# Moon0shang/HandPoseEstimation-with-3D-CNNs

Hardware: AMD Instinct MI355X
Metric: depth frames/sec to 32^3 TSDF (higher is better)
Workload: dtype f64

## Files before the change

handposeestimation-with-3d-cnns_amd/__init__.py:

```python
from . import _lib
from ._lib import TsdfCam, TsdfError, default_cam
from .voxelize import (AabbBatch, AugmentedStep, CloudGridBatch, MapGridBatch, ObbBatch, PointCloudBatch, PoseError, ProcessAugBatch, ProcessBatch, TsdfBatch,
                       aabb,
                       aug_state, aug_xforms, aug_xforms_at, cloud_grids, denormalize_joints, empty_batch,
                       frames_within, joints_within, normalize_joints, point_clouds, pose_error, process_batch, process_batch_aug,
                       project_joints, release_stream, transform_joints, voxel_pixels, voxelize_aug_grid,
                       voxelize, voxelize_aug, voxelize_grid, voxelize_indexed, voxelize_labels, widen_depth16,
                       invert_xforms, obb_xforms, voxelize_obb, narrow_volumes, voxelize_grid_lowp, voxelize_lowp,
                       map_grids, voxelize_aug_lowp, voxelize_map_grid_lowp, MapStepBatch, compose_xforms, map_step_head,
                       HandCrops, locate_hands, voxelize_frames)
from .pca import JointPCA, fit_joint_pca
from . import augment, dataset, export, packing, pca, shard, synth
from .dataset import MSRA_Dataset, MSRADepthDataset, ResidentLoader, VoxelBatch, VoxelLoader
from .tsdf_numba import cal_tsdf_cuda
from .tsdf_for import tsdf_cal, tsdf_f
from .process import DataProcess

__all__ = ["voxelize", "voxelize_labels", "voxelize_indexed", "ResidentLoader", "voxel_pixels", "release_stream", "voxelize_grid", "voxelize_aug", "augment", "aabb", "TsdfBatch", "AabbBatch", "TsdfCam", "TsdfError",
           "default_cam", "cal_tsdf_cuda", "tsdf_f", "tsdf_cal", "DataProcess", "packing", "shard",
           "synth", "dataset", "MSRADepthDataset", "MSRA_Dataset", "VoxelLoader", "VoxelBatch", "normalize_joints", "denormalize_joints",
           "pca", "JointPCA", "fit_joint_pca", "project_joints", "pose_error", "PoseError", "joints_within", "frames_within",
           "point_clouds", "PointCloudBatch", "cloud_grids", "CloudGridBatch", "process_batch", "ProcessBatch", "aug_xforms",
           "aug_xforms_at", "aug_state", "AugmentedStep", "voxelize_aug_grid", "transform_joints", "process_batch_aug",
           "ProcessAugBatch", "widen_depth16", "obb_xforms", "voxelize_obb", "invert_xforms", "ObbBatch",
           "voxelize_grid_lowp", "voxelize_lowp", "narrow_volumes", "map_grids", "MapGridBatch", "voxelize_map_grid_lowp",
           "voxelize_aug_lowp", "compose_xforms", "map_step_head", "MapStepBatch", "locate_hands", "voxelize_frames",
           "HandCrops"]
```

handposeestimation-with-3d-cnns_amd/_lib.py:

```python
from __future__ import annotations

import contextlib
import ctypes
import os
from typing import NamedTuple

_HERE = os.path.dirname(os.path.abspath(__file__))
_DEFAULT_LIB = os.path.join(_HERE, "libtsdf_hip.so")


def _lib_path() -> str:
    over = os.environ.get("TSDF_HIP_LIB")
    if not over or os.path.abspath(over) == _DEFAULT_LIB:
        return _DEFAULT_LIB
    if os.environ.get("TSDF_ALLOW_LIB_OVERRIDE") != "1":
        raise ImportError(f"TSDF_HIP_LIB={over} asks for a library other than {_DEFAULT_LIB}; set "
                          "TSDF_ALLOW_LIB_OVERRIDE=1 as well if that is intended (experiments only)")
    return over


LIB_PATH = _lib_path()

TSDF_LAYOUT_CZYX = 0
TSDF_LAYOUT_CXYZ = 1
LAYOUTS = {"czyx": TSDF_LAYOUT_CZYX, "cxyz": TSDF_LAYOUT_CXYZ}

TSDF_OK = 0
TSDF_FRAME_OK = 0
TSDF_FRAME_DEGENERATE = 1
TSDF_FRAME_BAD_HEADER = 2


class TsdfError(RuntimeError):
    """A tsdf_* entry point returned a negative status."""


class TsdfCam(ctypes.Structure):

    _fields_ = [
        ("focal", ctypes.c_double),
        ("cx", ctypes.c_double),
        ("cy", ctypes.c_double),
        ("invalid_eps", ctypes.c_float),
        ("trunc_voxels", ctypes.c_float),
    ]


class TsdfLabels(ctypes.Structure):

    _fields_ = [
        ("d_gt", ctypes.c_void_p),
        ("n_joints", ctypes.c_int),
        ("clamp", ctypes.c_int),
        ("d_out_gt_nor", ctypes.c_void_p),
        ("d_out_gt_aug", ctypes.c_void_p),
    ]


class TsdfPca(ctypes.Structure):

    _fields_ = [
        ("d_mean", ctypes.c_void_p),
        ("d_coeff", ctypes.c_void_p),
        ("n_components", ctypes.c_int),
        ("d_out_gt_pca", ctypes.c_void_p),
    ]


ABI_VERSION = 7
INLINE_INDEX_MAX = 32

DEBUG_LIB_PATH = os.path.join(os.path.dirname(_HERE), "build", "libtsdf_hip_debug.so")

AUGMENT_LIB_PATH = os.path.join(_HERE, "libtsdf_augment.so")
AUGMENT_VERSION = 1

AUGSTEP_LIB_PATH = os.path.join(_HERE, "libtsdf_augstep.so")
AUGSTEP_VERSION = 1

AUGGRID_LIB_PATH = os.path.join(_HERE, "libtsdf_auggrid.so")
AUGGRID_VERSION = 1

DEPTH16_LIB_PATH = os.path.join(_HERE, "libtsdf_depth16.so")
DEPTH16_VERSION = 1
DEPTH16_MAX_SHIFT = 7

OBB_LIB_PATH = os.path.join(_HERE, "libtsdf_obb.so")
OBB_VERSION = 1

LOWP_LIB_PATH = os.path.join(_HERE, "libtsdf_lowp.so")
LOWP_VERSION = 1
TSDF_LOWP_F16 = 1
TSDF_LOWP_BF16 = 2

MAPLOWP_LIB_PATH = os.path.join(_HERE, "libtsdf_maplowp.so")
MAPLOWP_VERSION = 1

MAPSTEP_LIB_PATH = os.path.join(_HERE, "libtsdf_mapstep.so")
MAPSTEP_VERSION = 1

LOCATE_LIB_PATH = os.path.join(_HERE, "libtsdf_locate.so")
LOCATE_VERSION = 1
TSDF_LOCATE_F32 = 0
TSDF_LOCATE_U16 = 1


class _Ext(NamedTuple):
    path: str
    version_symbol: str
    version: int
    entries: dict


_vp, _i, _i64, _u64 = ctypes.c_void_p, ctypes.c_int, ctypes.c_int64, ctypes.c_uint64

_EXTS = {
    "augment": _Ext(AUGMENT_LIB_PATH, "tsdf_augment_version", AUGMENT_VERSION, {
        "tsdf_aug_draw_hip": [_vp, _i64, _vp, _i, _u64, _u64, _vp, _vp, _vp, _vp],
    }),
    "augstep": _Ext(AUGSTEP_LIB_PATH, "tsdf_augstep_version", AUGSTEP_VERSION, {
        "tsdf_aug_draw_at_hip": [_vp, _i64, _vp, _i, _vp, _vp, _vp, _vp, _vp, _vp],
    }),
    "auggrid": _Ext(AUGGRID_LIB_PATH, "tsdf_auggrid_version", AUGGRID_VERSION, {
        "tsdf_voxelize_aug_grid_hip": [_vp, _i64, _vp, _vp, _i, _i, ctypes.POINTER(TsdfCam), _i, _vp, _vp, _vp, _vp, _vp],
        "tsdf_transform_joints_hip": [_vp, _vp, _i, _i, _vp, _vp],
    }),
    "depth16": _Ext(DEPTH16_LIB_PATH, "tsdf_depth16_version", DEPTH16_VERSION, {
        "tsdf_depth16_widen_hip": [_vp, _i64, _i, _vp, _vp],
        "tsdf_depth16_host_gather": [_vp, _i64, _vp, _i64, _vp, _i64, _vp, _i64, _vp, _i],
    }),
    "obb": _Ext(OBB_LIB_PATH, "tsdf_obb_version", OBB_VERSION, {
        "tsdf_obb_xforms_hip": [_vp, _i64, _vp, _vp, _i, ctypes.POINTER(TsdfCam), _vp, _vp, _vp, _vp],
    }),
    "lowp": _Ext(LOWP_LIB_PATH, "tsdf_lowp_version", LOWP_VERSION, {
        "tsdf_voxelize_grid_lowp_hip": [_vp, _i64, _vp, _vp, _i64, _vp, _i, _i, ctypes.POINTER(TsdfCam), _i, _i, _vp, _vp,
                                        _vp, _vp],
        "tsdf_lowp_narrow_hip": [_vp, _i64, _i, _vp, _vp],
    }),
    "maplowp": _Ext(MAPLOWP_LIB_PATH, "tsdf_maplowp_version", MAPLOWP_VERSION, {
        "tsdf_map_place_hip": [_vp, _i64, _vp, _vp, _i64, _vp, _i, _i, ctypes.POINTER(TsdfCam), _vp, _vp, _vp, _vp, _vp, _vp],
        "tsdf_voxelize_map_grid_lowp_hip": [_vp, _i64, _vp, _vp, _i64, _vp, _i, _i, ctypes.POINTER(TsdfCam), _i, _i, _vp, _vp,
                                            _vp, _vp, _vp],
    }),
    "mapstep": _Ext(MAPSTEP_LIB_PATH, "tsdf_mapstep_version", MAPSTEP_VERSION, {
        "tsdf_compose_xforms_hip": [_vp, _vp, _i64, _vp, _i, _vp, _vp],
        "tsdf_map_step_head_hip": [_vp, _i64, _vp, _vp, _i64, _vp, _i, _i, ctypes.c_double, ctypes.c_double, ctypes.c_double,
                                   ctypes.c_float, ctypes.c_float, _vp, _vp, _vp, _vp, _vp, _i, _i, _vp, _vp, _vp, _vp, _vp,
                                   _vp, _vp, _vp, _vp, _vp],
    }),
    "locate": _Ext(LOCATE_LIB_PATH, "tsdf_locate_version", LOCATE_VERSION, {
        "tsdf_locate_capacity": [_i, _i, ctypes.c_float, ctypes.c_float, ctypes.c_double, ctypes.POINTER(_i64)],
        "tsdf_locate_hip": [_vp, _i, _i, _i64, _i, _i, _vp, _i, ctypes.c_float, ctypes.c_float, ctypes.c_float,
                            ctypes.c_float, _i, _i, ctypes.c_double, ctypes.c_double, ctypes.c_double, ctypes.c_float,
                            ctypes.c_float, _i64, _vp, _vp, _vp, _vp, _vp, _vp, _vp, _vp, _vp, _vp],
    }),
}

_lib = None
_debug_lib = None
_ext_libs = {}


def _declare(L, entries: dict) -> None:
    for name, argtypes in entries.items():
        fn = getattr(L, name)
        fn.restype = ctypes.c_int
        fn.argtypes = argtypes


def _bind(L, path: str, debug: bool = False):
    vp = ctypes.c_void_p
    cam_p = ctypes.POINTER(TsdfCam)
    L.tsdf_version.restype = ctypes.c_int
    L.tsdf_version.argtypes = []
    if L.tsdf_version() != ABI_VERSION:
        raise ImportError(f"{path} has ABI version {L.tsdf_version()}, this package needs {ABI_VERSION}: rebuild it")
    L.tsdf_strerror.restype = ctypes.c_char_p
    L.tsdf_strerror.argtypes = [ctypes.c_int]
    L.tsdf_resolution_supported.restype = ctypes.c_int
    L.tsdf_resolution_supported.argtypes = [ctypes.c_int]
    L.tsdf_default_cam.restype = None
    L.tsdf_default_cam.argtypes = [cam_p]
    lab_p, pca_p = ctypes.POINTER(TsdfLabels), ctypes.POINTER(TsdfPca)
    i, i64 = ctypes.c_int, ctypes.c_int64
    pack = [vp, i64, vp, vp, i, i, cam_p, i, vp]
    indexed = [vp, i64, vp, vp, i64, vp, i, i, cam_p, i, vp]
    outs = [vp, vp, vp, vp]
    entries = {
            "tsdf_voxelize_hip": pack + outs,
            "tsdf_voxelize_labels_hip": pack + outs + [lab_p],
            "tsdf_voxelize_grid_hip": pack + [vp, vp, vp],
            "tsdf_voxelize_aug_hip": pack + [vp] + outs,
            "tsdf_voxelize_aug_labels_hip": pack + [vp] + outs + [lab_p],
            "tsdf_voxelize_labels_pca_hip": pack + [vp] + outs + [lab_p, pca_p],
            "tsdf_aabb_hip": pack[:7] + [vp] + [vp, vp, vp, vp],
            "tsdf_voxelize_indexed_hip": indexed + outs + [lab_p],
            "tsdf_voxelize_indexed_host_hip": indexed + outs + [lab_p],
            "tsdf_voxelize_indexed_aug_hip": indexed + [vp] + outs + [lab_p],
            "tsdf_voxelize_indexed_pca_hip": indexed + [vp] + outs + [lab_p, pca_p],
            "tsdf_voxelize_indexed_host_pca_hip": indexed + outs + [lab_p, pca_p],
            "tsdf_host_gather_frames": [vp, vp, i64, vp, i64, vp, i64, vp, i],
            "tsdf_host_gather_frames_n": [vp, i64, vp, i64, vp, i64, vp, i64, vp, i],
            "tsdf_normalize_joints_hip": [vp, vp, vp, i, i, i, vp, vp],
            "tsdf_denormalize_joints_hip": [vp, vp, vp, i, i, vp, vp],
            "tsdf_stream_release": [vp],
            "tsdf_project_joints_hip": [vp, vp, vp, i, i, pca_p, vp],
            "tsdf_pose_error_hip": [vp, pca_p, vp, vp, vp, i, i, vp, vp, vp, vp, vp],
            "tsdf_point_clouds_hip": pack[:4] + [i, i, cam_p, ctypes.c_uint64, i64, vp, vp, vp, vp, vp],
            "tsdf_cloud_grid_hip": [vp, i, i, i, cam_p, vp, vp, vp, vp, vp, vp],
            "tsdf_describe_launch": [i, i, i, i, ctypes.c_char_p, i],
            "tsdf_debug_pixmap_hip": pack + [vp, vp, vp, vp],
            "tsdf_debug_set_queue_word": [vp, ctypes.c_uint64],
    }
    _declare(L, {k: v for k, v in entries.items() if debug or not k.startswith("tsdf_debug_")})
    return L


def load():
    global _lib
    if _lib is not None:
        return _lib
    if not os.path.exists(LIB_PATH):
        raise ImportError(
            f"{LIB_PATH} not found: build it with `python -c 'import __graft_entry__ as g; g.build()'` "
            "or `make -C handposeestimation-with-3d-cnns_amd/csrc`. There is no CPU fallback."
        )
    _lib = _bind(ctypes.CDLL(LIB_PATH), LIB_PATH)
    return _lib


def load_debug():
    global _debug_lib
    if _debug_lib is not None:
        return _debug_lib
    if not os.path.exists(DEBUG_LIB_PATH):
        raise ImportError(f"{DEBUG_LIB_PATH} not found: build it with `make -C handposeestimation-with-3d-cnns_amd/csrc debug` "
                          "(__graft_entry__.build() does)")
    L = _bind(ctypes.CDLL(DEBUG_LIB_PATH), DEBUG_LIB_PATH, debug=True)
    _debug_lib = L
    return L


def _load_ext(name: str):
    L = _ext_libs.get(name)
    if L is not None:
        return L
    ext = _EXTS[name]
    if not os.path.exists(ext.path):
        raise ImportError(f"{ext.path} not found: build it with `make -C handposeestimation-with-3d-cnns_amd/csrc "
                          f"{name}` (__graft_entry__.build() does). There is no CPU fallback.")
    L = ctypes.CDLL(ext.path)
    _declare(L, {ext.version_symbol: [], **ext.entries})
    have = getattr(L, ext.version_symbol)()
    if have != ext.version:
        raise ImportError(f"{ext.path} has version {have}, this package needs {ext.version}: rebuild it")
    _ext_libs[name] = L
    return L


def load_augment():
    return _load_ext("augment")


def load_augstep():
    return _load_ext("augstep")


def load_auggrid():
    return _load_ext("auggrid")


def load_depth16():
    return _load_ext("depth16")


def load_obb():
    return _load_ext("obb")


def load_lowp():
    return _load_ext("lowp")


def load_maplowp():
    return _load_ext("maplowp")


def load_mapstep():
    return _load_ext("mapstep")


def load_locate():
    return _load_ext("locate")


@contextlib.contextmanager
def using_debug_library():
    global _lib
    prev = _lib
    _lib = load_debug()
    try:
        yield _lib
    finally:
        _lib = prev


def check(status: int, what: str):
    if status != TSDF_OK:
        msg = load().tsdf_strerror(status).decode()
        raise TsdfError(f"{what}: {msg} (status {status})")


def default_cam() -> TsdfCam:
    c = TsdfCam()
    load().tsdf_default_cam(ctypes.byref(c))
    return c
```

handposeestimation-with-3d-cnns_amd/dataset.py:

```python
from __future__ import annotations

import ctypes
import os
import sys
import queue
import threading
import warnings
from typing import Iterator, List, NamedTuple, Optional, Sequence, Tuple, Union

import numpy as np
import torch
import torch.utils.data as data

from . import _lib, augment, packing, shard
from .pca import JointPCA, fit_joint_pca
from .voxelize import (AugmentedStep, TsdfBatch, _get_raw_stream, aabb, aug_state, aug_xforms, aug_xforms_at,
                       denormalize_joints, empty_batch, normalize_joints, obb_xforms, project_joints, voxelize,
                       voxelize_aug, voxelize_grid_lowp, voxelize_indexed, voxelize_labels, widen_depth16, _lowp_dtype)


def _common_depth_shift(packs: Sequence[packing.PackedFrames]) -> Optional[int]:
    forms = sorted({-1 if pk.depth_shift is None else int(pk.depth_shift) for pk in packs})
    if len(forms) > 1:
        names = ", ".join("float32" if f < 0 else f"16-bit with shift {f}" for f in forms)
        raise ValueError(f"the packs of one dataset must share one depth form, these are {names}: repack them "
                         "(packing.pack_tree(..., depth16=None) or one forced shift, overwrite=True)")
    return None if not forms or forms[0] < 0 else forms[0]


def _subset(size: str) -> Tuple[int, int]:
    if size == "full":
        return 9, 17
    if size == "small":
        return 4, 5
    raise ValueError("size must be 'full' or 'small'")


class MSRADepthDataset(data.Dataset):

    def __init__(self, root_path: str, train: bool = True, test_idx: int = 2, size: str = "full",
                 subjects: Optional[Sequence[str]] = None, packed_dir: Optional[str] = None,
                 build_packs: bool = True):
        n_sub, n_ges = _subset(size)
        self.root_path = root_path
        self.train = train
        self.test_idx = test_idx
        if subjects is not None:
            all_sub = list(subjects)
        elif root_path is not None and os.path.isdir(root_path):
            skip = os.path.abspath(packed_dir) if packed_dir is not None else None
            all_sub = sorted(d for d in os.listdir(root_path) if os.path.isdir(os.path.join(root_path, d))
                             and os.path.abspath(os.path.join(root_path, d)) != skip)[:n_sub]
        elif packed_dir is not None:
            all_sub = sorted(f[:-7] for f in os.listdir(packed_dir) if f.endswith(".tsdfpk"))[:n_sub]
        else:
            raise ValueError("root_path is not a directory and no packed_dir was given")
        if not 0 <= test_idx < len(all_sub):
            raise ValueError("test_idx out of range")
        chosen = [s for i, s in enumerate(all_sub) if (i != test_idx) == train]
        self.subjects = chosen
        self.paths: List[str] = []
        self.packs: List[packing.PackedFrames] = []
        self._pack_of = np.zeros(0, np.int32)
        self._local = np.zeros(0, np.int64)
        gts: List[np.ndarray] = []
        if packed_dir is not None:
            pk_of, loc = [], []
            for sub in chosen:
                path = os.path.join(packed_dir, sub + ".tsdfpk")
                if not os.path.exists(path):
                    if not build_packs:
                        raise FileNotFoundError(path)
                    packing.pack_tree(root_path, packed_dir, subjects=[sub])
                pk = packing.PackedFrames.load(path, mmap=True)
                gs = pk.group_start if pk.group_start is not None else np.array([0, len(pk)])
                end = int(gs[min(n_ges, len(gs) - 1)])
                self.packs.append(pk)
                pk_of.append(np.full(end, len(self.packs) - 1, np.int32))
                loc.append(np.arange(end, dtype=np.int64))
                gts.append(np.asarray(pk.gt[:end]) if pk.gt is not None else np.zeros((end, 63), np.float32))
            if pk_of:
                self._pack_of, self._local = np.concatenate(pk_of), np.concatenate(loc)
        else:
            for sub in chosen:
                sub_dir = os.path.join(root_path, sub)
                gestures = sorted(g for g in os.listdir(sub_dir) if os.path.isdir(os.path.join(sub_dir, g)))
                for ges in gestures[:n_ges]:
                    g_dir = os.path.join(sub_dir, ges)
                    bin_num, gt = packing.read_joint(g_dir)
                    self.paths += packing.gesture_bin_paths(g_dir, bin_num)
                    gts.append(gt)
        self.depth_shift = _common_depth_shift(self.packs)
        self.ground_truth = np.concatenate(gts) if gts else np.zeros((0, 63), np.float32)

    @classmethod
    def from_packs(cls, packs: Sequence[packing.PackedFrames]) -> "MSRADepthDataset":
        self = cls.__new__(cls)
        self.root_path, self.train, self.test_idx, self.subjects, self.paths = None, True, -1, [], []
        self.packs = list(packs)
        self.depth_shift = _common_depth_shift(self.packs)
        self._pack_of = np.concatenate([np.full(len(pk), k, np.int32) for k, pk in enumerate(self.packs)])
        self._local = np.concatenate([np.arange(len(pk), dtype=np.int64) for pk in self.packs])
        self.ground_truth = np.concatenate([np.asarray(pk.gt) if pk.gt is not None else np.zeros((len(pk), 63), np.float32)
                                            for pk in self.packs])
        return self

    @property
    def packed(self) -> bool:
        return bool(self.packs)

    def __len__(self) -> int:
        return len(self._local) if self.packed else len(self.paths)

    def pixels(self) -> Optional[np.ndarray]:
        if not self.packed:
            return None
        out = np.empty(len(self), np.int64)
        for k, pk in enumerate(self.packs):
            m = self._pack_of == k
            out[m] = pk.pixels[self._local[m]]
        return out

    def __getitem__(self, index: int):
        if self.packed:
            pk = self.packs[int(self._pack_of[index])]
            h, d = pk.frame(int(self._local[index]))
            return np.asarray(h), np.asarray(d), self.ground_truth[index]
        header, depth = packing.read_bin(self.paths[index])
        return header, depth, self.ground_truth[index]

    def pin_packs(self, limit_bytes: int = 32 << 30) -> bool:
        if not self.packed or sum(int(pk.depth.nbytes) for pk in self.packs) > limit_bytes:
            return False
        for pk in self.packs:
            pk.pin()
        return True

    def contiguous_source(self, idx: np.ndarray):
        idx = np.asarray(idx, np.int64)
        if not self.packed or idx.size == 0 or not (np.diff(idx) == 1).all():
            return None
        ks = self._pack_of[idx]
        pk = self.packs[int(ks[0])]
        if ks[0] != ks[-1] or getattr(pk, "_pinned", None) is None:
            return None
        a, b = int(self._local[idx[0]]), int(self._local[idx[-1]]) + 1
        view = pk.slice(a, b)
        view.gt = self.ground_truth[idx]
        return pk._pinned[int(pk.offsets[a]):int(pk.offsets[b])], view

    def take(self, idx: np.ndarray, depth_out: Optional[np.ndarray] = None) -> packing.PackedFrames:
        idx = np.asarray(idx, np.int64)
        if self.packed and idx.size:
            ks = self._pack_of[idx]
            if (ks == ks[0]).all():
                out = self.packs[int(ks[0])].take(self._local[idx], depth_out)
                out.gt = self.ground_truth[idx]
                return out
            if self.depth_shift is not None:
                raw = [self.packs[int(k)].raw_frame(int(l)) for k, l in zip(ks, self._local[idx])]
                off = np.zeros(idx.size + 1, np.int64)
                np.cumsum([d.size for _, d in raw], out=off[1:])
                if depth_out is not None and depth_out.dtype != np.uint16:
                    raise TypeError(f"depth_out is {depth_out.dtype}, the dataset's packs hold uint16 depth")
                depth = depth_out[: off[-1]] if depth_out is not None else np.empty(int(off[-1]), np.uint16)
                for k, (_, d) in enumerate(raw):
                    depth[off[k]:off[k + 1]] = d
                return packing.PackedFrames(depth, off, np.stack([np.asarray(h) for h, _ in raw]), self.ground_truth[idx],
                                            depth_shift=self.depth_shift)
            pk = packing.pack_frames(self.packs[int(k)].frame(int(l)) for k, l in zip(ks, self._local[idx]))
            if depth_out is not None:
                depth_out[: pk.depth.size] = pk.depth
                pk.depth = depth_out[: pk.depth.size]
            pk.gt = self.ground_truth[idx]
            return pk
        pk = packing.pack_frames(self[int(i)][:2] for i in idx)
        if depth_out is not None:
            depth_out[: pk.depth.size] = pk.depth
            pk.depth = depth_out[: pk.depth.size]
        pk.gt = self.ground_truth[idx] if idx.size else np.zeros((0, 63), np.float32)
        return pk


def collate_frames(batch) -> Tuple[packing.PackedFrames, np.ndarray]:
    pk = packing.pack_frames((h, d) for h, d, _ in batch)
    gt = np.stack([g for _, _, g in batch]).astype(np.float32) if batch else np.zeros((0, 63), np.float32)
    return pk, gt


def voxelize_batch(pk: packing.PackedFrames, gt: np.ndarray, device, res: int = 32, pin: bool = True):
    depth, offsets, headers = pk.to_torch(device, pin=pin, non_blocking=True)
    tgt = torch.from_numpy(np.ascontiguousarray(gt))
    if pin:
        tgt = tgt.pin_memory()
    tgt = tgt.to(device, non_blocking=True)
    out: TsdfBatch = voxelize(depth, offsets, headers, res=res)
    return out.tsdf, tgt, out.max_l, out.mid_p, out.status


class VoxelBatch(NamedTuple):

    tsdf: torch.Tensor
    gt: torch.Tensor
    max_l: torch.Tensor
    mid_p: torch.Tensor
    status: torch.Tensor
    gt_nor: Optional[torch.Tensor]


def plan_batches(n: int, batch_size: int, rank: int = 0, world: int = 1, shuffle: bool = False, seed: int = 0,
                 epoch: int = 0, drop_last: bool = False, weights: Optional[np.ndarray] = None,
                 balance: Optional[str] = None) -> List[np.ndarray]:
    if balance is None:
        balance = "pixels" if weights is not None else "frames"
    if balance not in ("frames", "pixels"):
        raise ValueError("balance must be 'frames' or 'pixels'")
    if balance == "pixels" and weights is None:
        raise ValueError("balance='pixels' needs the per-frame weights")
    bounds = shard.shard_bounds(n, world, weights if balance == "pixels" else None)
    if not 0 <= rank < world:
        raise ValueError("rank out of range")
    a, b = bounds[rank]
    idx = np.arange(a, b, dtype=np.int64)
    if shuffle:
        np.random.default_rng((seed, epoch, rank)).shuffle(idx)
    if balance == "frames":
        if n < world:
            raise ValueError(f"balance='frames' needs at least one frame per rank (n={n}, world={world})")
        lens = [e - s for s, e in bounds]
        if not drop_last and idx.size < max(lens):
            idx = np.concatenate([idx, idx[:1]])
    batches = [idx[i:i + batch_size] for i in range(0, idx.size, batch_size)]
    if balance == "frames":
        if drop_last:
            batches = batches[: min(lens) // batch_size]
    elif drop_last and batches and batches[-1].size < batch_size:
        batches.pop()
    return batches


class _Staging:

    def __init__(self, max_px: int, bs: int, device, with_gt: bool, depth16: bool = False):
        self.h_depth = torch.empty(max_px, dtype=torch.uint16 if depth16 else torch.float32).pin_memory()
        self.d_depth16 = torch.empty(max_px, dtype=torch.uint16, device=device) if depth16 else None
        self.h_off = torch.empty(bs + 1, dtype=torch.int64).pin_memory()
        self.h_hdr = torch.empty((bs, 6), dtype=torch.int32).pin_memory()
        self.h_gt = torch.empty((bs, 63), dtype=torch.float32).pin_memory() if with_gt else None
        self.d_depth = torch.empty(max_px, dtype=torch.float32, device=device)
        self.copied = torch.cuda.Event()
        self.consumed = torch.cuda.Event()
        self.filled = threading.Event()
        self.free = threading.Event()
        self.free.set()
        self.used = False
        self.n = 0
        self.npx = 0
        self.src = None


class _BatchLoader:

    def __init__(self, dataset: MSRADepthDataset, batch_size: int, device, res, shuffle, seed, drop_last, rank, world,
                 labels, clamp, layout, balance):
        self.balance = balance
        self.ds, self.bs, self.device, self.res = dataset, int(batch_size), torch.device(device), res
        self.shuffle, self.seed, self.drop_last = shuffle, seed, drop_last
        self.rank, self.world = rank, world
        self.labels, self.clamp, self.layout = labels, clamp, layout
        self.epoch = 0

    def _batches(self) -> List[np.ndarray]:
        return plan_batches(len(self.ds), self.bs, self.rank, self.world, self.shuffle, self.seed, self.epoch,
                            self.drop_last, self.ds.pixels() if self.balance == "pixels" else None, self.balance)

    def __len__(self) -> int:
        return len(self._batches())


class VoxelLoader(_BatchLoader):

    def __init__(self, dataset: MSRADepthDataset, batch_size: int, device, res: int = 32,
                 shuffle: bool = False, seed: int = 0, drop_last: bool = False,
                 rank: int = 0, world: int = 1, labels: bool = True, clamp: bool = True,
                 max_pixels: Optional[int] = None, layout: str = "czyx", pin_packs: bool = True,
                 balance: str = "frames"):
        super().__init__(dataset, batch_size, device, res, shuffle, seed, drop_last, rank, world, labels, clamp, layout,
                         balance)
        self.max_px = int(max_pixels) if max_pixels else self.bs * 320 * 240
        self.pin_packs = pin_packs
        self._sets: Optional[List[_Staging]] = None
        self._copy_stream = None

    def __iter__(self) -> Iterator[VoxelBatch]:
        batches = self._batches()
        self.epoch += 1
        if self._sets is None:
            self._sets = [_Staging(self.max_px, self.bs, self.device, True, getattr(self.ds, "depth_shift", None) is not None)
                          for _ in range(2)]
            if self.pin_packs:
                self.ds.pin_packs()
        sets = self._sets
        shift = getattr(self.ds, "depth_shift", None)
        for s in sets:
            if s.used:
                s.consumed.synchronize()
            s.free.set()
            s.filled.clear()
            s.used = False
        err: "queue.Queue" = queue.Queue()
        stop = threading.Event()

        def work():
            try:
                for k, b in enumerate(batches):
                    s = sets[k & 1]
                    while not s.free.wait(0.05):
                        if stop.is_set():
                            return
                    s.free.clear()
                    if s.used:
                        s.consumed.synchronize()
                    direct = self.ds.contiguous_source(b)
                    if direct is not None:
                        s.src, pk = direct
                    else:
                        pk = self.ds.take(b, s.h_depth.numpy())
                        s.src = s.h_depth[: pk.depth.size]
                    if pk.depth.size > self.max_px:
                        raise ValueError(f"batch of {pk.depth.size} pixels exceeds max_pixels={self.max_px}")
                    s.n, s.npx = len(pk), int(pk.depth.size)
                    s.h_off.numpy()[: s.n + 1] = pk.offsets
                    s.h_hdr.numpy()[: s.n] = pk.headers
                    s.h_gt.numpy()[: s.n] = pk.gt
                    s.filled.set()
            except BaseException as e:
                err.put(e)
                for s in sets:
                    s.filled.set()

        t = threading.Thread(target=work, daemon=True)
        t.start()
        if self._copy_stream is None:
            self._copy_stream = torch.cuda.Stream(device=self.device)
        copy_stream = self._copy_stream
        try:
            for k in range(len(batches)):
                cur = torch.cuda.current_stream(self.device)
                s = sets[k & 1]
                s.filled.wait()
                if not err.empty():
                    raise err.get()
                s.filled.clear()
                n, npx = s.n, s.npx
                with torch.cuda.stream(copy_stream):
                    if k >= 2:
                        copy_stream.wait_event(s.consumed)
                    if shift is None:
                        s.d_depth[:npx].copy_(s.src, non_blocking=True)
                    else:
                        s.d_depth16[:npx].copy_(s.src, non_blocking=True)
                        widen_depth16(s.d_depth16[:npx], shift, out=s.d_depth[:npx])
                    s.copied.record(copy_stream)
                cur.wait_event(s.copied)
                out, gt_nor, gt = voxelize_labels(s.d_depth[:npx], s.h_off[: n + 1], s.h_hdr[:n], s.h_gt[:n], res=self.res,
                                                  layout=self.layout, clamp=self.clamp, gt_copy=True)
                if not self.labels:
                    gt_nor = None
                s.consumed.record(cur)
                s.used = True
                s.free.set()
                yield VoxelBatch(out.tsdf, gt, out.max_l, out.mid_p, out.status, gt_nor)
        finally:
            stop.set()
            t.join()


class ResidentPacks:

    def __init__(self, dataset: MSRADepthDataset, device):
        if not dataset.packed:
            raise ValueError("a resident dataset needs packs (packing.pack_tree + packed_dir=, or from_packs)")
        packs = dataset.packs
        px = np.array([int(pk.depth.size) for pk in packs], np.int64)
        nf = np.array([len(pk) for pk in packs], np.int64)
        pbase = np.concatenate([[0], np.cumsum(px)])
        fbase = np.concatenate([[0], np.cumsum(nf)])
        self.depth = torch.empty(int(pbase[-1]), dtype=torch.float32, device=device)
        with warnings.catch_warnings():
            warnings.simplefilter("ignore", UserWarning)
            for k, pk in enumerate(packs):
                dst = self.depth[int(pbase[k]):int(pbase[k + 1])]
                if pk.depth_shift is None:
                    dst.copy_(torch.from_numpy(np.ascontiguousarray(pk.depth)))
                else:
                    tmp = torch.from_numpy(np.ascontiguousarray(pk.depth)).to(self.depth.device)
                    widen_depth16(tmp, pk.depth_shift, out=dst)
                    del tmp
        off = np.concatenate([np.asarray(pk.offsets[:-1], np.int64) + pbase[k] for k, pk in enumerate(packs)]
                             + [pbase[-1:]])
        hdr = np.concatenate([np.asarray(pk.headers, np.int32).reshape(-1, 6) for pk in packs])
        gt = np.concatenate([np.asarray(pk.gt, np.float32).reshape(len(pk), -1) if pk.gt is not None
                             else np.zeros((len(pk), 63), np.float32) for pk in packs])
        self.offsets = torch.from_numpy(off).to(device)
        self.headers = torch.from_numpy(np.ascontiguousarray(hdr)).to(device)
        self.gt = torch.from_numpy(np.ascontiguousarray(gt)).to(device)
        self.frame = fbase[dataset._pack_of] + dataset._local

    def nbytes(self) -> int:
        return 4 * self.depth.numel()


class ResidentLoader(_BatchLoader):

    def __init__(self, dataset: MSRADepthDataset, batch_size: int, device, res: int = 32, shuffle: bool = False,
                 seed: int = 0, drop_last: bool = False, rank: int = 0, world: int = 1, labels: bool = True,
                 clamp: bool = True, layout: str = "czyx", augment: Union[bool, str] = False, balance: str = "frames",
                 prefetch: int = 1, ring: int = 2, graph: bool = False, frame: str = "camera",
                 volume_dtype: Optional[torch.dtype] = None):
        if frame not in ("camera", "obb"):
            raise ValueError(f"frame must be 'camera' or 'obb', got {frame!r}")
        if frame == "obb" and (augment or graph):
            raise ValueError("frame='obb' does not combine with augment or graph=True (the two maps are not composed)")
        if volume_dtype is not None:
            _lowp_dtype(volume_dtype)
            if augment or graph or frame == "obb":
                raise ValueError("volume_dtype does not combine with augment, frame='obb' or graph=True (the low-precision "
                                 "voxel pass is the plain one)")
        if not dataset.packed:
            raise ValueError("ResidentLoader needs a pack-backed dataset (packing.pack_tree + packed_dir=, or from_packs)")
        if prefetch < 1 or ring < 2:
            raise ValueError("prefetch must be >= 1 and ring >= 2")
        if isinstance(augment, str) and augment != "device":
            raise ValueError(f"augment must be False, True or 'device', got {augment!r}")
        if graph is not False and graph is not True:
            raise ValueError(f"graph must be False or True, got {graph!r}")
        if graph and (augment != "device" or prefetch != 1):
            raise ValueError("graph=True replays the augmented step: it needs augment='device' and prefetch=1")
        self.augment = bool(augment)
        self.device_draws = augment == "device"
        self.graph = graph
        self.frame = frame
        self.obb = None
        self.obb_status = None
        self._step = None
        self.volume_dtype = volume_dtype
        self._lowp = None
        self._lowp_ring = None
        self._mapped = self.augment or frame == "obb"
        self.prefetch, self.ring = int(prefetch), int(ring)
        super().__init__(dataset, batch_size, device, res, shuffle, seed, drop_last, rank, world, labels, clamp, layout,
                         balance)
        self._dev = None
        self._g = None
        self._idx = None
        self._blocks = None

    def resident_bytes(self) -> int:
        return sum(4 * int(pk.depth.size) for pk in self.ds.packs)

    def _upload(self):
        rp = ResidentPacks(self.ds, self.device)
        self._dev = (rp.depth, rp.offsets, rp.headers, rp.gt)
        self._g = rp.frame
        pin = self.bs > _lib.INLINE_INDEX_MAX or self._mapped
        self._idx = [(torch.empty(self.bs, dtype=torch.int64).pin_memory() if pin else torch.empty(self.bs, dtype=torch.int64),
                      torch.cuda.Event()) for _ in range(2)]
        self._used = [False, False]
        self._mid = None
        if self.frame == "obb":
            ob = obb_xforms(rp.depth, rp.offsets, rp.headers)
            self.obb, self.obb_status = ob.xforms, ob.status
        if self.volume_dtype is not None:
            ab = aabb(rp.depth, rp.offsets, rp.headers, res=self.res)
            rows = torch.cat([ab.ori, ab.grid[:, 4:6], torch.zeros_like(ab.ori)], dim=1)
            self._lowp = (rows, ab.grid[:, 3].contiguous(), ab.grid[:, :3].contiguous(), ab.status)
        if self.augment:
            mid = aabb(rp.depth, rp.offsets, rp.headers, res=self.res).grid[:, :3]
            if self.device_draws:
                self._mid = mid.contiguous()
                self._xf = torch.empty((self.ring if self.prefetch > 1 else 2, self.bs * self.prefetch, 24),
                                       dtype=torch.float64, device=self.device)
            else:
                self._mid = mid.cpu().numpy().astype(np.float64)
                self._xf = [torch.empty((self.bs, 24), dtype=torch.float64).pin_memory() for _ in range(2)]

    def __iter__(self) -> Iterator[VoxelBatch]:
        batches = self._batches()
        self.epoch += 1
        if self._dev is None:
            self._upload()
        if self.volume_dtype is not None:
            return self._iter_lowp(batches)
        if self.prefetch > 1:
            return self._iter_blocks(batches, self.epoch)
        return self._iter_single(batches, self.epoch)

    def _iter_lowp(self, batches) -> Iterator[VoxelBatch]:
        depth, off, hdr, gt = self._dev
        rows, max_l, mid_p, status = self._lowp
        if not batches:
            return
        bs, P, R = self.bs, self.prefetch, self.res
        if P > 1 and self._lowp_ring is None:
            self._lowp_ring = [torch.empty((bs * P, 3, R, R, R), dtype=self.volume_dtype, device=self.device)
                               for _ in range(self.ring)]
        d_idx = torch.from_numpy(np.ascontiguousarray(self._g[np.concatenate(batches)])).to(self.device)
        pos = 0
        for blk, k0 in enumerate(range(0, len(batches), P)):
            mine = batches[k0:k0 + P]
            nfr = int(sum(b.size for b in mine))
            idx = d_idx[pos:pos + nfr]
            pos += nfr
            out = self._lowp_ring[blk % self.ring][:nfr] if P > 1 else None
            tsdf, _ = voxelize_grid_lowp(depth, off, hdr, rows, res=R, layout=self.layout, dtype=self.volume_dtype,
                                         index=idx, out=out)
            ml, mp, st = max_l.index_select(0, idx), mid_p.index_select(0, idx), status.index_select(0, idx)
            g = gt.index_select(0, idx)
            gt_nor = None
            if self.labels:
                gt_nor = normalize_joints(g, ml, mp, clamp=self.clamp)
                bad = (st != _lib.TSDF_FRAME_OK).reshape((-1,) + (1,) * (g.dim() - 1))
                gt_nor = torch.where(bad, torch.full_like(gt_nor, 0.5), gt_nor)
            a = 0
            for b in mine:
                e = a + int(b.size)
                yield VoxelBatch(tsdf[a:e], g[a:e], ml[a:e], mp[a:e], st[a:e], gt_nor[a:e] if self.labels else None)
                a = e

    def _epoch_key(self, epoch: int) -> int:
        return augment.device_key(self.seed, epoch, self.rank) if self.device_draws else 0

    def _host_draw(self, gidx: np.ndarray, batches, epoch: int, k0: int = 0) -> np.ndarray:
        xf = np.empty((gidx.size, 24), np.float64)
        pos = 0
        for k, b in enumerate(batches, k0):
            xf[pos:pos + b.size] = augment.random_affines(self._mid[gidx[pos:pos + b.size]],
                                                          rng=(self.seed, epoch, self.rank, k))[0]
            pos += b.size
        return xf

    def _maps(self, index: torch.Tensor, slot: int, key: int, pos: int, drawn: Optional[torch.Tensor]):
        if self.frame == "obb":
            return self.obb.index_select(0, index)
        if self.device_draws:
            return aug_xforms(self._mid, index=index, key=key, counter0=pos, out=self._xf[slot, :index.numel()])
        return drawn

    def _iter_single(self, batches, epoch) -> Iterator[VoxelBatch]:
        depth, off, hdr, gt = self._dev
        key, pos = self._epoch_key(epoch), 0
        for k, b in enumerate(batches):
            cur = torch.cuda.current_stream(self.device)
            h_idx, done = self._idx[k & 1]
            if self._used[k & 1]:
                done.synchronize()
            n = int(b.size)
            gidx = self._g[b]
            if self.graph and n == self.bs:
                if self._step is None:
                    self._step = AugmentedStep(depth, off, hdr, n, gt=gt, centres=self._mid, res=self.res,
                                               layout=self.layout, clamp=self.clamp)
                out, gt_nor, g = self._step.step(gidx, key, pos)
            else:
                h_idx.numpy()[:n] = gidx
                xf, idx = None, h_idx[:n]
                if self._mapped:
                    drawn = None
                    if self.frame == "obb":
                        idx = idx.to(self.device, non_blocking=True)
                    elif not self.device_draws:
                        h_xf = self._xf[k & 1]
                        h_xf.numpy()[:n] = self._host_draw(gidx, (b,), epoch, k)
                        drawn = h_xf[:n].to(self.device, non_blocking=True)
                    xf = self._maps(idx, k & 1, key, pos, drawn)
                out, gt_nor, g = voxelize_indexed(depth, off, hdr, idx, gt, res=self.res, layout=self.layout,
                                                  clamp=self.clamp, gt_copy=True, xforms=xf)
                done.record(cur)
                self._used[k & 1] = True
            pos += n
            yield VoxelBatch(out.tsdf, g, out.max_l, out.mid_p, out.status, gt_nor if self.labels else None)

    def _make_blocks(self):
        depth, off, hdr, gt = self._dev
        cap, R = self.bs * self.prefetch, self.res
        lab_shape = (cap,) + tuple(gt.shape[1:])
        blocks = []
        for _ in range(self.ring):
            out = empty_batch(cap, R, self.device)
            gt_nor = torch.empty(lab_shape, dtype=torch.float32, device=self.device)
            g = torch.empty(lab_shape, dtype=torch.float32, device=self.device)
            views = [self._view(out, gt_nor, g, j * self.bs, (j + 1) * self.bs) for j in range(self.prefetch)]
            blocks.append((out, gt_nor, g, views))
        return blocks

    def _view(self, out, gt_nor, g, a, b) -> VoxelBatch:
        return VoxelBatch(out.tsdf[a:b], g[a:b], out.max_l[a:b], out.mid_p[a:b], out.status[a:b],
                          gt_nor[a:b] if self.labels else None)

    def _iter_blocks(self, batches, epoch) -> Iterator[VoxelBatch]:
        depth, off, hdr, gt = self._dev
        if self._blocks is None:
            self._blocks = self._make_blocks()
        if not batches:
            return
        bs, P = self.bs, self.prefetch
        flat = np.concatenate(batches)
        gidx = self._g[flat]
        d_idx = torch.from_numpy(np.ascontiguousarray(gidx)).to(self.device)
        key = self._epoch_key(epoch)
        d_xf = None
        if self.augment and not self.device_draws:
            d_xf = torch.from_numpy(self._host_draw(gidx, batches, epoch)).to(self.device)
        pos = 0
        for blk, k0 in enumerate(range(0, len(batches), P)):
            mine = batches[k0:k0 + P]
            nfr = int(sum(b.size for b in mine))
            out, gt_nor, g, views = self._blocks[blk % self.ring]
            full = nfr == bs * P
            if full:
                o, gn, gg = out, gt_nor, g
            else:
                o = TsdfBatch(out.tsdf[:nfr], out.max_l[:nfr], out.mid_p[:nfr], out.status[:nfr])
                gn, gg = gt_nor[:nfr], g[:nfr]
            idx, xf = d_idx[pos:pos + nfr], None
            if self._mapped:
                xf = self._maps(idx, blk % self.ring, key, pos, None if d_xf is None else d_xf[pos:pos + nfr])
            voxelize_indexed(depth, off, hdr, idx, gt, res=self.res, layout=self.layout, clamp=self.clamp,
                             out=o, out_gt_nor=gn, out_gt=gg, xforms=xf)
            pos += nfr
            if full:
                yield from views
            else:
                a = 0
                for b in mine:
                    yield self._view(out, gt_nor, g, a, a + int(b.size))
                    a += int(b.size)


class PreBatched:

    __slots__ = ("batch",)

    def __init__(self, batch):
        self.batch = batch


def _collate_prebatched(batch, *, collate_fn_map=None):
    return batch[0].batch


try:
    from torch.utils.data._utils.collate import default_collate_fn_map as _collate_map
    _collate_map[PreBatched] = _collate_prebatched
except ImportError:
    _collate_map = None


class _SlotGuard:

    __slots__ = ("batch", "_stor", "_cdata", "_base")

    def __init__(self, batch):
        self.batch = batch
        self._stor = tuple(t.untyped_storage() for t in batch)
        self._cdata = tuple(s._cdata for s in self._stor)
        self._base = None

    def counts(self):
        rc, uc, b, c = sys.getrefcount, _storage_use_count, self.batch, self._cdata
        if len(c) == 5:
            return (rc(b), rc(b[0]), rc(b[1]), rc(b[2]), rc(b[3]), rc(b[4]), uc(c[0]), uc(c[1]), uc(c[2]), uc(c[3]),
                    uc(c[4]))
        return (rc(b), rc(b[0]), rc(b[1]), rc(b[2]), rc(b[3]), uc(c[0]), uc(c[1]), uc(c[2]), uc(c[3]))

    def arm(self):
        self._base = self.counts()

    def held(self) -> bool:
        return self.counts() != self._base


_storage_use_count = getattr(torch._C, "_storage_Use_Count", None)
_guard_ok: Optional[bool] = None


def _slot_guard_works() -> bool:
    global _guard_ok
    if _guard_ok is None:
        ok = _storage_use_count is not None
        if ok:
            try:
                holder = [PreBatched(tuple(torch.zeros(2, 3) for _ in range(4)))]
                g = _SlotGuard(holder[0].batch)
                g.arm()
                ok = not g.held()
                for make in (lambda b: b, lambda b: b[1], lambda b: b[0][:, 1], lambda b: b[2].detach(), lambda b: b[3].data,
                             lambda b: b[0].numpy()):
                    ref = make(holder[0].batch)
                    ok = ok and g.held()
                    del ref
                    ok = ok and not g.held()
            except Exception:
                ok = False
        _guard_ok = bool(ok)
    return _guard_ok


class MSRA_Dataset(data.Dataset):

    def __init__(self, root_path, opt=None, train=True, aug=False, device="cuda", block: int = 1024,
                 packed_dir: Optional[str] = None, resident: Optional[bool] = None, prebatched: Optional[bool] = None,
                 ring: Optional[int] = None, aug_seed: int = 0, _raw: Optional[MSRADepthDataset] = None, pca=None):
        if isinstance(aug, str) and aug != "device":
            raise ValueError(f"aug must be False, True or 'device', got {aug!r}")
        self.AUG = bool(aug)
        self.aug_device = aug == "device"
        self.aug_seed = aug_seed
        self.size = getattr(opt, "size", "small")
        self.test_idx = int(getattr(opt, "test_index", 2))
        self.PCA_SZ = int(getattr(opt, "PCA_SZ", 63))
        self.train = train
        self.raw = _raw if _raw is not None else MSRADepthDataset(root_path, train=train, test_idx=self.test_idx,
                                                                  size=self.size, packed_dir=packed_dir)
        self.device = torch.device(device)
        self.block = int(block)
        self._cache_block = -1
        self._cache: Optional[TsdfBatch] = None
        self._cache_gt: Optional[torch.Tensor] = None
        self._last = -1
        self.resident = self.raw.packed if resident is None else bool(resident)
        self.prebatched = (self.resident and _collate_map is not None) if prebatched is None else bool(prebatched)
        if self.prebatched and not self.resident:
            raise ValueError("prebatched=True needs a resident (pack-backed) dataset")
        self._ring_req = ring
        self._rp: Optional[ResidentPacks] = None
        self._fast = None
        self._n = len(self.raw)
        self._aug_params = None
        self._xf_table = None
        self._aug_key = 0
        self._aug_state = None
        self._aug_mid = None
        if self.aug_device:
            self._aug_key = augment.device_key(aug_seed, 0, 0)
        elif self.AUG:
            self._aug_params = augment.draw_params(self._n, aug_seed)
        self.pca = None
        self._cache_pca: Optional[torch.Tensor] = None
        if pca is not None and pca is not False:
            if pca is True:
                if not train:
                    raise ValueError("pca=True fits on a TRAINING dataset; pass the training set's basis (its .pca, a "
                                     "JointPCA or a path) to a test dataset")
                basis = fit_joint_pca(self)
            elif isinstance(pca, JointPCA):
                basis = pca
            else:
                basis = JointPCA.load(os.fspath(pca))
            basis.check_k(self.PCA_SZ)
            self.pca = basis.to(self.device)
            self.PCA_mean, self.PCA_coeff = basis.torch_decode_args(self.PCA_SZ, self.device)

    @classmethod
    def from_raw(cls, raw: MSRADepthDataset, device="cuda", **kw) -> "MSRA_Dataset":
        return cls(None, device=device, _raw=raw, **kw)

    def __len__(self):
        return 2 * self._n if self.AUG else self._n

    def _resident_packs(self) -> "ResidentPacks":
        if self._rp is None:
            self._rp = ResidentPacks(self.raw, self.device)
            if self.AUG:
                rp = self._rp
                mid = aabb(rp.depth, rp.offsets, rp.headers).grid[:, :3]
                self._frame2 = np.ascontiguousarray(np.concatenate([rp.frame, rp.frame]))
                if self.aug_device:
                    self._aug_mid = mid.contiguous()
                    self._draw_frame = np.ascontiguousarray(np.concatenate([np.full(self._n, -1, np.int64), rp.frame]))
                    self._draw_counter = np.ascontiguousarray(np.tile(np.arange(self._n, dtype=np.int64), 2))
                else:
                    mid = mid.cpu().numpy().astype(np.float64)[rp.frame]
                    self._xf_table = np.ascontiguousarray(np.concatenate(
                        [augment.identity_affines(self._n), augment.affines_from_params(mid, *self._aug_params)]))
        return self._rp

    def _device_state(self) -> torch.Tensor:
        if self._aug_state is None:
            self._aug_state = aug_state(self._aug_key, 0, self.device)
        return self._aug_state

    def _device_maps(self, idx: np.ndarray) -> torch.Tensor:
        return aug_xforms_at(self._aug_mid, self._device_state(),
                             index=torch.from_numpy(self._draw_frame[idx]).to(self.device),
                             counters=torch.from_numpy(self._draw_counter[idx]).to(self.device))

    def _voxelize_items(self, idx: np.ndarray, clamp: bool = True):
        dev = self.device
        kw = {} if self.pca is None else {"pca": self.pca, "k": self.PCA_SZ}
        if self.resident:
            rp = self._resident_packs()
            xf = None
            if self.aug_device:
                xf = self._device_maps(idx)
            elif self.AUG:
                xf = torch.from_numpy(self._xf_table[idx]).to(dev)
            frame = self._frame2 if self.AUG else rp.frame
            r = voxelize_indexed(rp.depth, rp.offsets, rp.headers, torch.from_numpy(frame[idx]).to(dev), rp.gt,
                                 clamp=clamp, gt_copy=True, xforms=xf, **kw)
            return r[0], r[2], r[1], (r[3] if kw else None)
        src = idx % self._n
        pk = self.raw.take(src)
        depth, offsets, headers = pk.to_torch(dev, pin=False, non_blocking=False)
        gt = torch.from_numpy(np.ascontiguousarray(pk.gt)).to(dev)
        if not self.AUG:
            if not kw:
                return voxelize(depth, offsets, headers, res=32), gt, None, None
            out, gt_nor, gt_pca = voxelize_labels(depth, offsets, headers, gt, res=32, clamp=clamp, **kw)
            return out, gt, gt_nor, gt_pca
        mid = aabb(depth, offsets, headers).grid[:, :3]
        if self.aug_device:
            pos = np.where(idx < self._n, -1, np.arange(idx.size)).astype(np.int64)
            xf = aug_xforms_at(mid.contiguous(), self._device_state(), index=torch.from_numpy(pos).to(dev),
                               counters=torch.from_numpy(np.ascontiguousarray(src, np.int64)).to(dev))
        else:
            xf = augment.affines_from_params(mid.cpu().numpy().astype(np.float64), *(p[src] for p in self._aug_params))
            plain = idx < self._n
            xf[plain] = augment.identity_affines(int(plain.sum()))
            xf = torch.from_numpy(xf).to(dev)
        out, gt_nor, gt_aug = voxelize_aug(depth, offsets, headers, xf, res=32, gt=gt, clamp=clamp)
        gt_pca = project_joints(gt_aug, out.max_l, out.mid_p, self.pca, self.PCA_SZ) if kw else None
        return out, gt_aug, gt_nor, gt_pca

    def _fit_labels(self) -> np.ndarray:
        n, dev, us = self._n, self.device, []
        if self.resident:
            rp = self._resident_packs()
            ab = aabb(rp.depth, rp.offsets, rp.headers)
            fr = torch.from_numpy(rp.frame).to(dev)
            grid, st, gt = ab.grid[fr], ab.status[fr], rp.gt[fr]
            u = normalize_joints(gt.contiguous(), grid[:, 3].contiguous(), grid[:, :3].contiguous(), clamp=False)
            us.append(u[st == 0].cpu().numpy())
        else:
            for a in range(0, n, self.block):
                pk = self.raw.take(np.arange(a, min(n, a + self.block)))
                depth, offsets, headers = pk.to_torch(dev, pin=False, non_blocking=False)
                ab = aabb(depth, offsets, headers)
                gt = torch.from_numpy(np.ascontiguousarray(pk.gt)).to(dev)
                u = normalize_joints(gt, ab.grid[:, 3].contiguous(), ab.grid[:, :3].contiguous(), clamp=False)
                us.append(u[ab.status == 0].cpu().numpy())
        for a in range(n, len(self), self.block):
            out, _, u, _ = self._voxelize_items(np.arange(a, min(len(self), a + self.block)), clamp=False)
            us.append(u[out.status == 0].cpu().numpy())
        return np.concatenate(us) if us else np.zeros((0, 63), np.float32)

    def _tuples(self, out, gt, gt_pca, m: int):
        if gt_pca is None:
            return [(out.tsdf[k], gt[k], out.max_l[k], out.mid_p[k]) for k in range(m)]
        return [(out.tsdf[k], gt[k], out.max_l[k], out.mid_p[k], gt_pca[k]) for k in range(m)]

    def _load_block(self, blk: int):
        a, b = blk * self.block, min(len(self.raw), (blk + 1) * self.block)
        self._cache, self._cache_gt, _, self._cache_pca = self._voxelize_items(np.arange(a, b))
        self._cache_block = blk

    class _Fast:

        kGroup = 16
        pca, k = None, 0

        def __init__(self, rp: "ResidentPacks", bs: int, ring: int, device, frame=None, xf_table=None, pca=None, k=0,
                     draw=None):
            self._ctypes, self._lib = ctypes, _lib
            self.always_fresh = not _slot_guard_works()
            ring = max(2, int(ring))
            self.iring = -(-max(ring, self.kGroup) // self.kGroup) * self.kGroup
            self.bs, self.ring, self.count, self.replaced = bs, ring, 0, 0
            self.L = _lib.load()
            self.pca, self.k = pca, int(k)
            self.rp_gt = rp.gt
            self.nc = rp.gt.shape[1]
            d = torch.device(device)
            self.device = d if d.index is not None else torch.device("cuda", torch.cuda.current_device())
            self.dev_index = self.device.index
            self.h_idx = torch.empty((self.iring, bs), dtype=torch.int64).pin_memory()
            self.h_idx_np = self.h_idx.numpy()
            self.rows = [self.h_idx_np[k] for k in range(self.iring)]
            self.idx_ptrs = [self.h_idx[k].data_ptr() for k in range(self.iring)]
            self.head = (rp.depth.data_ptr(), rp.depth.numel(), rp.offsets.data_ptr(), rp.headers.data_ptr(),
                         int(rp.headers.shape[0]))
            self.slots = [None] * ring
            self.labels = [None] * ring
            self.args = [None] * ring
            self.pcas = [None] * ring
            self.results = [None] * ring
            self.guard = [None] * ring
            for k in range(ring):
                self._fresh(k)
            self.read = [torch.cuda.Event() for _ in range(self.iring // self.kGroup)]
            self.read_used = [False] * (self.iring // self.kGroup)
            self.raw_stream = _get_raw_stream if _get_raw_stream is not None else \
                (lambda i: torch.cuda.current_stream(i).cuda_stream)
            self.cur_dev = getattr(torch._C, "_cuda_getDevice", torch.cuda.current_device)
            self.fn = self.L.tsdf_voxelize_indexed_hip
            self.plain_xf = ()
            if pca is not None:
                self.fn, self.plain_xf = self.L.tsdf_voxelize_indexed_pca_hip, (None,)
            self.take = (rp.frame if frame is None else frame).take
            self.by_value = xf_table is None and draw is None and bs <= _lib.INLINE_INDEX_MAX
            self.fn_host = self.L.tsdf_voxelize_indexed_host_hip if pca is None else \
                self.L.tsdf_voxelize_indexed_host_pca_hip
            self.fn_aug = self.L.tsdf_voxelize_indexed_aug_hip if pca is None else self.L.tsdf_voxelize_indexed_pca_hip
            self.idx_buf = np.empty(bs, np.int64)
            self.idx_ptr = self.idx_buf.ctypes.data
            self.xf_take = None
            if xf_table is not None:
                self.h_xf = torch.empty((self.iring, bs, 24), dtype=torch.float64).pin_memory()
                self.h_xf_np = self.h_xf.numpy()
                self.xf_rows = [self.h_xf_np[k] for k in range(self.iring)]
                self.xf_ptr = [self.h_xf[k].data_ptr() for k in range(self.iring)]
                self.xf_take = xf_table.take
            self.draw = None
            if draw is not None:
                centres, state, frames, counters = draw
                self.fn_draw = _lib.load_augstep().tsdf_aug_draw_at_hip
                self.draw = (centres, state)
                self.draw_head = (centres.data_ptr(), int(centres.shape[0]))
                self.state_ptr = state.data_ptr()
                self.h_draw = torch.empty((self.iring, 2, bs), dtype=torch.int64).pin_memory()
                self.h_draw_np = self.h_draw.numpy()
                self.draw_rows = [(self.h_draw_np[k, 0], self.h_draw_np[k, 1]) for k in range(self.iring)]
                self.draw_ptrs = [(self.h_draw[k, 0].data_ptr(), self.h_draw[k, 1].data_ptr()) for k in range(self.iring)]
                self.d_xf = torch.empty((self.iring, bs, 24), dtype=torch.float64, device=self.device)
                self.xf_ptr = [self.d_xf[k].data_ptr() for k in range(self.iring)]
                self.frame_take, self.counter_take = frames.take, counters.take

        def _fresh(self, k: int) -> None:
            self._alloc(k)
            self.guard[k].arm()

        def _alloc(self, k: int) -> None:
            R, bs, nc, dev = 32, self.bs, self.nc, self.device
            tsdf = torch.empty((bs, 3, R, R, R), dtype=torch.float32, device=dev)
            gt = torch.empty((bs, nc), dtype=torch.float32, device=dev)
            max_l = torch.empty(bs, dtype=torch.float32, device=dev)
            mid_p = torch.empty((bs, 3), dtype=torch.float32, device=dev)
            status = torch.empty(bs, dtype=torch.int32, device=dev)
            gt_nor = torch.empty((bs, nc), dtype=torch.float32, device=dev)
            self.slots[k] = (tsdf, gt, max_l, mid_p, status, gt_nor)
            self.labels[k] = self._lib.TsdfLabels(self.rp_gt.data_ptr(), nc // 3, 1, gt_nor.data_ptr(), gt.data_ptr())
            self.args[k] = (tsdf.data_ptr(), max_l.data_ptr(), mid_p.data_ptr(), status.data_ptr(),
                            self._ctypes.byref(self.labels[k]))
            batch = (tsdf, gt, max_l, mid_p)
            if self.pca is not None:
                gt_pca = torch.empty((bs, self.k), dtype=torch.float32, device=dev)
                mean, coeff = self.pca.device_tensors(dev)
                self.pcas[k] = self._lib.TsdfPca(mean.data_ptr(), coeff.data_ptr(), self.k, gt_pca.data_ptr())
                self.slots[k] = self.slots[k] + (gt_pca,)
                self.args[k] = self.args[k] + (self._ctypes.byref(self.pcas[k]),)
                batch = batch + (gt_pca,)
            self.results[k] = [PreBatched(batch)]
            self.guard[k] = _SlotGuard(self.results[k][0].batch)

        def held(self, k: int) -> bool:
            return self.always_fresh or self.guard[k].held()

        def next_slot(self) -> int:
            k = self.count % self.ring
            if self.held(k):
                self._fresh(k)
                self.replaced += 1
            return k

        def sync(self) -> None:
            torch.cuda.current_stream(self.device).synchronize()

    def _ring_size(self, n: int) -> int:
        if self._ring_req:
            return max(2, int(self._ring_req))
        vol = n * (3 * 32 ** 3 * 4)
        return max(2, min(256, (2 << 30) // max(vol, 1)))

    def _fast_batch(self, indices):
        f = self._fast
        n = len(indices)
        if f is None or n > f.bs:
            if f is not None:
                f.sync()
            f = self._fast = MSRA_Dataset._Fast(self._rp, n, self._ring_size(n), self.device,
                                                frame=self._frame2 if self.AUG else None, xf_table=self._xf_table,
                                                pca=self.pca, k=self.PCA_SZ,
                                                draw=(self._aug_mid, self._device_state(), self._draw_frame,
                                                      self._draw_counter) if self.aug_device else None)
        k = f.next_slot()
        a = f.args[k]
        if f.by_value:
            fn = f.fn_host
            f.idx_buf[:n] = f.take(indices)
            with torch.cuda.device(f.device):
                rc = fn(*f.head, f.idx_ptr, n, 32, None, 0, f.raw_stream(f.dev_index), *a)
        else:
            ki = f.count % f.iring
            within = ki & (f.kGroup - 1)
            if within == 0 and f.read_used[ki >> 4]:
                f.read[ki >> 4].synchronize()
            if n == f.bs:
                f.take(indices, out=f.rows[ki])
            else:
                f.h_idx_np[ki, :n] = f.take(indices)
            if f.draw is not None:
                fr, cn = f.draw_rows[ki]
                if n == f.bs:
                    f.frame_take(indices, out=fr)
                    f.counter_take(indices, out=cn)
                else:
                    fr[:n] = f.frame_take(indices)
                    cn[:n] = f.counter_take(indices)
                with torch.cuda.device(f.device):
                    stream = f.raw_stream(f.dev_index)
                    fn = f.fn_draw
                    rc = fn(*f.draw_head, f.draw_ptrs[ki][0], n, f.state_ptr, f.draw_ptrs[ki][1], stream, f.xf_ptr[ki],
                            None, None)
                    if rc == 0:
                        fn = f.fn_aug
                        rc = fn(*f.head, f.idx_ptrs[ki], n, 32, None, 0, stream, f.xf_ptr[ki], *a)
            elif f.xf_take is not None:
                fn = f.fn_aug
                if n == f.bs:
                    f.xf_take(indices, axis=0, out=f.xf_rows[ki])
                else:
                    f.h_xf_np[ki, :n] = f.xf_take(indices, axis=0)
                with torch.cuda.device(f.device):
                    rc = fn(*f.head, f.idx_ptrs[ki], n, 32, None, 0, f.raw_stream(f.dev_index), f.xf_ptr[ki], *a)
            else:
                fn = f.fn
                if f.cur_dev() == f.dev_index:
                    rc = fn(*f.head, f.idx_ptrs[ki], n, 32, None, 0, f.raw_stream(f.dev_index), *f.plain_xf, *a)
                else:
                    with torch.cuda.device(f.device):
                        rc = fn(*f.head, f.idx_ptrs[ki], n, 32, None, 0, f.raw_stream(f.dev_index), *f.plain_xf, *a)
            if within == f.kGroup - 1:
                f.read[ki >> 4].record(torch.cuda.current_stream(f.device))
                f.read_used[ki >> 4] = True
        if rc != 0:
            _lib.check(rc, fn.__name__)
        f.count += 1
        if n == f.bs:
            return f.results[k]
        return [PreBatched(tuple(t[:n] for t in f.results[k][0].batch))]

    def __getitems__(self, indices):
        if data.get_worker_info() is not None:
            raise RuntimeError("MSRA_Dataset produces its items on the GPU: use it with num_workers=0 (the reference's "
                               "default, train.py:38), there is nothing for loader processes to do")
        f = self._fast
        if f is not None and f.by_value and len(indices) == f.bs and f.cur_dev() == f.dev_index:
            k = f.next_slot()
            f.take(indices, out=f.idx_buf)
            a = f.args[k]
            rc = f.fn_host(*f.head, f.idx_ptr, f.bs, 32, None, 0, f.raw_stream(f.dev_index), *a)
            if rc != 0:
                _lib.check(rc, "tsdf_voxelize_indexed_host_hip")
            f.count += 1
            self._last = indices[-1]
            return f.results[k]
        if self.prebatched:
            if not indices:
                raise IndexError("empty batch")
            self._resident_packs()
            self._last = indices[-1]
            return self._fast_batch(indices)
        idx = np.asarray([int(i) for i in indices], np.int64)
        if idx.size and (idx.min() < 0 or idx.max() >= len(self)):
            raise IndexError(int(idx.max() if idx.max() >= len(self) else idx.min()))
        self._last = int(idx[-1]) if idx.size else self._last
        out, gt, _, gt_pca = self._voxelize_items(idx)
        return self._tuples(out, gt, gt_pca, idx.size)

    def _items_of(self, indices):
        r = self.__getitems__(indices)
        if r and isinstance(r[0], PreBatched):
            b = r[0].batch
            return [tuple(t[k].clone() for t in b) for k in range(len(indices))]
        return r

    def __getitem__(self, index):
        index = int(index)
        if not 0 <= index < len(self):
            raise IndexError(index)
        if self.AUG:
            self._last = index
            return self._items_of([index])[0]
        blk = index // self.block
        if blk != self._cache_block:
            if index != self._last + 1 and index % self.block:
                return self._items_of([index])[0]
            self._load_block(blk)
        self._last = index
        k = index - blk * self.block
        c = self._cache
        if self._cache_pca is not None:
            return c.tsdf[k], self._cache_gt[k], c.max_l[k], c.mid_p[k], self._cache_pca[k]
        return c.tsdf[k], self._cache_gt[k], c.max_l[k], c.mid_p[k]
```

handposeestimation-with-3d-cnns_amd/voxelize.py:

```python
from __future__ import annotations

import ctypes
from typing import NamedTuple, Optional

import torch

from . import _lib


class TsdfBatch(NamedTuple):
    tsdf: torch.Tensor
    max_l: torch.Tensor
    mid_p: torch.Tensor
    status: torch.Tensor


_get_raw_stream = getattr(torch._C, "_cuda_getCurrentRawStream", None)


def _raw_stream(dev) -> int:
    if _get_raw_stream is not None:
        return _get_raw_stream(dev.index)
    return torch.cuda.current_stream(dev).cuda_stream


class _Current:

    __slots__ = ("guard",)

    def __init__(self, dev):
        self.guard = None if torch.cuda.current_device() == dev.index else torch.cuda.device(dev)

    def __enter__(self):
        if self.guard is not None:
            self.guard.__enter__()

    def __exit__(self, *exc):
        if self.guard is not None:
            self.guard.__exit__(*exc)
        return False


def _dev_check(name, t, dtype, device=None, host_ok=False):
    if t.__class__ is torch.Tensor and t.is_cuda and t.dtype is dtype and t.is_contiguous() and \
            (device is None or t.device == device):
        return
    if not isinstance(t, torch.Tensor):
        raise TypeError(f"{name} must be a torch.Tensor")
    if host_ok and not t.is_cuda and t.is_pinned():
        device = None
    elif not t.is_cuda:
        raise ValueError(f"{name} must live on the GPU" + (" or in page-locked host memory" if host_ok else "") +
                         f" (there is no CPU path); got device {t.device}")
    if t.dtype != dtype:
        raise TypeError(f"{name} must be {dtype}, got {t.dtype}")
    if not t.is_contiguous():
        raise ValueError(f"{name} must be contiguous")
    if device is not None and t.device != device:
        raise ValueError(f"{name} is on {t.device}, expected {device}")


def _pack(L, depth, offsets, headers, res=None, layout="czyx"):
    if layout not in _lib.LAYOUTS:
        raise ValueError("layout must be 'czyx' or 'cxyz'")
    _dev_check("depth", depth, torch.float32)
    dev = depth.device
    _dev_check("offsets", offsets, torch.int64, dev, host_ok=True)
    _dev_check("headers", headers, torch.int32, dev, host_ok=True)
    if headers.dim() != 2 or headers.shape[1] != 6:
        raise ValueError("headers must have shape [n, 6]")
    n = headers.shape[0]
    if offsets.numel() != n + 1:
        raise ValueError("offsets must have n+1 entries")
    if res is None:
        return dev, n, None
    if not L.tsdf_resolution_supported(int(res)):
        raise ValueError(f"unsupported grid resolution {res} (multiple of 4 in 4..128)")
    return dev, n, int(res)


def _coords(name, t, rows) -> int:
    if t.shape[0] != rows:
        raise ValueError(f"{name} must have shape [{rows}, 3*J] or [{rows}, J, 3]")
    nc = t.numel() // rows if rows else 0
    if rows and (nc % 3 or not 1 <= nc // 3 <= 170):
        raise ValueError(f"{name} must hold 1..170 joints of 3 coordinates per frame")
    return nc


def _shaped(name, t, shape, dtype, dev):
    _dev_check(name, t, dtype, dev)
    if tuple(t.shape) != shape and (len(shape) != 1 or t.numel() != shape[0]):
        raise ValueError(f"{name} must have shape {shape}")
    return t


def _out(name, t, shape, dtype, dev):
    return torch.empty(shape, dtype=dtype, device=dev) if t is None else _shaped(name, t, shape, dtype, dev)


def empty_batch(n: int, R: int, dev) -> TsdfBatch:
    return TsdfBatch(_out("tsdf", None, (n, 3, R, R, R), torch.float32, dev), _out("max_l", None, (n,), torch.float32, dev),
                     _out("mid_p", None, (n, 3), torch.float32, dev), _out("status", None, (n,), torch.int32, dev))


def _make_out(out, n, R, dev) -> "TsdfBatch":
    if out is None:
        return empty_batch(n, R, dev)
    _dev_check("out.tsdf", out.tsdf, torch.float32, dev)
    _dev_check("out.max_l", out.max_l, torch.float32, dev)
    _dev_check("out.mid_p", out.mid_p, torch.float32, dev)
    _dev_check("out.status", out.status, torch.int32, dev)
    if tuple(out.tsdf.shape) != (n, 3, R, R, R) or out.max_l.numel() != n or \
            tuple(out.mid_p.shape) != (n, 3) or out.status.numel() != n:
        raise ValueError("out tensors have the wrong shape")
    return out


def _cam(cam):
    return ctypes.byref(cam) if cam is not None else None


def _ptr(t):
    return t.data_ptr() if t is not None else None


def _head(depth, offsets, headers, n, R, cam, layout) -> list:
    return [depth.data_ptr(), depth.numel(), offsets.data_ptr(), headers.data_ptr(), n, R, _cam(cam), _lib.LAYOUTS[layout],
            None]


def _call(dev, fn, args: list, stream_at: int) -> None:
    with _Current(dev):
        args[stream_at] = _raw_stream(dev)
        rc = fn(*args)
    _lib.check(rc, fn.__name__)


def _labels_struct(gt, n_src, n, dev, clamp, out_gt_nor=None, out_gt=None, want_gt=False):
    _dev_check("gt", gt, torch.float32, dev, host_ok=True)
    nc = _coords("gt", gt, n_src) or 63
    shape = (n,) + tuple(gt.shape[1:])
    gt_nor = _out("out_gt_nor", out_gt_nor, shape, torch.float32, dev)
    gt_dev = _out("out_gt", out_gt, shape, torch.float32, dev) if want_gt or out_gt is not None else None
    return _lib.TsdfLabels(gt.data_ptr(), nc // 3, 1 if clamp else 0, gt_nor.data_ptr(), _ptr(gt_dev)), gt_nor, gt_dev


def voxelize(depth: torch.Tensor, offsets: torch.Tensor, headers: torch.Tensor, res: int = 32,
             layout: str = "czyx", cam: Optional[_lib.TsdfCam] = None,
             out: Optional[TsdfBatch] = None) -> TsdfBatch:
    L = _lib.load()
    dev, n, R = _pack(L, depth, offsets, headers, res, layout)
    out = _make_out(out, n, R, dev)
    if n:
        _call(dev, L.tsdf_voxelize_hip, _head(depth, offsets, headers, n, R, cam, layout) +
              [out.tsdf.data_ptr(), out.max_l.data_ptr(), out.mid_p.data_ptr(), out.status.data_ptr()], 8)
    return out


def voxelize_labels(depth: torch.Tensor, offsets: torch.Tensor, headers: torch.Tensor, gt: torch.Tensor,
                    res: int = 32, layout: str = "czyx", cam: Optional[_lib.TsdfCam] = None, clamp: bool = True,
                    out: Optional[TsdfBatch] = None, out_gt_nor: Optional[torch.Tensor] = None,
                    gt_copy: bool = False, pca=None, k: Optional[int] = None):
    L = _lib.load()
    dev, n, R = _pack(L, depth, offsets, headers, res, layout)
    out = _make_out(out, n, R, dev)
    lab, gt_nor, gt_dev = _labels_struct(gt, n, n, dev, clamp, out_gt_nor, want_gt=gt_copy)
    pst = gt_pca = None
    if pca is not None:
        pst, gt_pca = _pca_struct(pca, k, n, lab.n_joints, dev)
    if n:
        head = _head(depth, offsets, headers, n, R, cam, layout)
        tail = [out.tsdf.data_ptr(), out.max_l.data_ptr(), out.mid_p.data_ptr(), out.status.data_ptr(), ctypes.byref(lab)]
        if pst is None:
            _call(dev, L.tsdf_voxelize_labels_hip, head + tail, 8)
        else:
            _call(dev, L.tsdf_voxelize_labels_pca_hip, head + [None] + tail + [ctypes.byref(pst)], 8)
    return ((out, gt_nor, gt_dev) if gt_copy else (out, gt_nor)) + ((gt_pca,) if pca is not None else ())


def voxelize_indexed(depth: torch.Tensor, offsets: torch.Tensor, headers: torch.Tensor, index: torch.Tensor,
                     gt: Optional[torch.Tensor] = None, res: int = 32, layout: str = "czyx",
                     cam: Optional[_lib.TsdfCam] = None, clamp: bool = True, out: Optional[TsdfBatch] = None,
                     gt_copy: bool = False, xforms: Optional[torch.Tensor] = None,
                     out_gt_nor: Optional[torch.Tensor] = None, out_gt: Optional[torch.Tensor] = None,
                     pca=None, k: Optional[int] = None):
    L = _lib.load()
    by_value = isinstance(index, torch.Tensor) and not index.is_cuda and not index.is_pinned() and \
        index.dtype is torch.int64 and index.dim() == 1 and index.is_contiguous() and \
        index.numel() <= _lib.INLINE_INDEX_MAX and xforms is None
    if not by_value:
        _dev_check("index", index, torch.int64, depth.device if isinstance(depth, torch.Tensor) else None, host_ok=True)
    if index.dim() != 1:
        raise ValueError("index must have shape [n]")
    dev, n_pack, R = _pack(L, depth, offsets, headers, res, layout)
    n = index.numel()
    out = _make_out(out, n, R, dev)
    lab = gt_nor = gt_dev = None
    if xforms is not None:
        _dev_check("xforms", xforms, torch.float64, dev, host_ok=True)
        if xforms.numel() != 24 * n:
            raise ValueError("xforms must have shape [n, 24] (forward rows then inverse rows)")
    if gt is not None:
        _dev_check("gt", gt, torch.float32, dev, host_ok=True)
        if gt.dim() < 2:
            raise ValueError("gt must hold the labels of every frame of the pack: [N, 3*J] or [N, J, 3]")
        lab, gt_nor, gt_dev = _labels_struct(gt, n_pack, n, dev, clamp, out_gt_nor, out_gt, want_gt=gt_copy)
        gt_copy = gt_dev is not None
    pst = gt_pca = None
    if pca is not None:
        if gt is None:
            raise ValueError("pca= needs gt (the projection is of the batch's labels)")
        pst, gt_pca = _pca_struct(pca, k, n, lab.n_joints, dev)
    if n:
        head = _head(depth, offsets, headers, n, R, cam, layout)
        head[4:5] = [n_pack, index.data_ptr(), n]
        tail = [out.tsdf.data_ptr(), out.max_l.data_ptr(), out.mid_p.data_ptr(), out.status.data_ptr(),
                ctypes.byref(lab) if lab is not None else None]
        if pst is not None:
            if by_value:
                _call(dev, L.tsdf_voxelize_indexed_host_pca_hip, head + tail + [ctypes.byref(pst)], 10)
            else:
                _call(dev, L.tsdf_voxelize_indexed_pca_hip, head + [_ptr(xforms)] + tail + [ctypes.byref(pst)], 10)
        elif by_value:
            _call(dev, L.tsdf_voxelize_indexed_host_hip, head + tail, 10)
        elif xforms is None:
            _call(dev, L.tsdf_voxelize_indexed_hip, head + tail, 10)
        else:
            _call(dev, L.tsdf_voxelize_indexed_aug_hip, head + [xforms.data_ptr()] + tail, 10)
    if gt is None:
        return out
    return ((out, gt_nor, gt_dev) if gt_copy else (out, gt_nor)) + ((gt_pca,) if pca is not None else ())


def _pca_struct(pca, k, n, n_joints, dev, out=None):
    k = pca.check_k(k)
    if pca.n_coords != 3 * n_joints:
        raise ValueError(f"the PCA basis is for {pca.n_coords} coordinates, the labels have {3 * n_joints}")
    mean, coeff = pca.device_tensors(dev)
    out = _out("out", out, (n, k), torch.float32, dev)
    return _lib.TsdfPca(mean.data_ptr(), coeff.data_ptr(), k, out.data_ptr()), out


def _frames(name, x, max_l, mid_p):
    _dev_check(name, x, torch.float32)
    dev, n = x.device, x.shape[0]
    _dev_check("max_l", max_l, torch.float32, dev)
    _dev_check("mid_p", mid_p, torch.float32, dev)
    if max_l.numel() != n or tuple(mid_p.shape) != (n, 3):
        raise ValueError("max_l must be [n] and mid_p [n,3]")
    return dev, n


def project_joints(gt: torch.Tensor, max_l: torch.Tensor, mid_p: torch.Tensor, pca, k: Optional[int] = None,
                   out: Optional[torch.Tensor] = None) -> torch.Tensor:
    L = _lib.load()
    dev, n = _frames("gt", gt, max_l, mid_p)
    nc = _coords("gt", gt, n) or pca.n_coords
    pst, out = _pca_struct(pca, k, n, nc // 3, dev, out)
    if n:
        _call(dev, L.tsdf_project_joints_hip, [gt.data_ptr(), max_l.data_ptr(), mid_p.data_ptr(), n, nc // 3,
                                               ctypes.byref(pst), None], 6)
    return out


class PoseError(NamedTuple):
    err: torch.Tensor
    frame_mean: torch.Tensor
    frame_max: torch.Tensor
    joints: Optional[torch.Tensor]


def pose_error(pred: torch.Tensor, gt: torch.Tensor, max_l: torch.Tensor, mid_p: torch.Tensor, pca=None,
               joints: bool = False) -> PoseError:
    L = _lib.load()
    _dev_check("pred", pred, torch.float32)
    dev = pred.device
    n = pred.shape[0]
    _dev_check("gt", gt, torch.float32, dev)
    _dev_check("max_l", max_l, torch.float32, dev)
    _dev_check("mid_p", mid_p, torch.float32, dev)
    if gt.shape[0] != n or max_l.numel() != n or tuple(mid_p.shape) != (n, 3):
        raise ValueError("pred, gt, max_l [n] and mid_p [n,3] must describe the same n frames")
    nc = _coords("gt", gt, n) or (pca.n_coords if pca is not None else 63)
    nj = nc // 3
    pst = None
    if pca is not None:
        if pred.dim() != 2:
            raise ValueError("pred must be [n, K] PCA coefficients")
        k = pca.check_k(pred.shape[1])
        if pca.n_coords != nc:
            raise ValueError(f"the PCA basis is for {pca.n_coords} coordinates, gt has {nc}")
        mean, coeff = pca.device_tensors(dev)
        pst = _lib.TsdfPca(mean.data_ptr(), coeff.data_ptr(), k, None)
    elif pred.numel() != n * nc:
        raise ValueError("pred must hold 3*J normalised coordinates per frame (or pass pca=)")
    res = PoseError(_out("err", None, (n, nj), torch.float32, dev), _out("frame_mean", None, (n,), torch.float32, dev),
                    _out("frame_max", None, (n,), torch.float32, dev),
                    _out("joints", None, (n, nc), torch.float32, dev) if joints else None)
    if n:
        _call(dev, L.tsdf_pose_error_hip,
              [pred.data_ptr(), ctypes.byref(pst) if pst is not None else None, max_l.data_ptr(), mid_p.data_ptr(),
               gt.data_ptr(), n, nj, None, res.err.data_ptr(), res.frame_mean.data_ptr(), res.frame_max.data_ptr(),
               _ptr(res.joints)], 7)
    return res


def joints_within(err: torch.Tensor, mm: float = 20.0) -> torch.Tensor:
    return (err < mm).sum().to(torch.float32) / err.numel() * 100


def frames_within(err: torch.Tensor, mm: float) -> torch.Tensor:
    return (err.amax(dim=1) <= mm).to(torch.float32).mean()


def normalize_joints(gt: torch.Tensor, max_l: torch.Tensor, mid_p: torch.Tensor, clamp: bool = True,
                     out: Optional[torch.Tensor] = None) -> torch.Tensor:
    return _norm_call(gt, max_l, mid_p, clamp, False, out)


def denormalize_joints(pred: torch.Tensor, max_l: torch.Tensor, mid_p: torch.Tensor,
                       out: Optional[torch.Tensor] = None) -> torch.Tensor:
    return _norm_call(pred, max_l, mid_p, False, True, out)


def _norm_call(x, max_l, mid_p, clamp, inverse, out):
    L = _lib.load()
    dev, n = _frames("joints", x, max_l, mid_p)
    nc = _coords("joints", x, n) or 63
    out = _out("out", out, tuple(x.shape), torch.float32, dev)
    if n:
        args = [x.data_ptr(), max_l.data_ptr(), mid_p.data_ptr(), n, nc // 3]
        if inverse:
            _call(dev, L.tsdf_denormalize_joints_hip, args + [None, out.data_ptr()], 5)
        else:
            _call(dev, L.tsdf_normalize_joints_hip, args + [1 if clamp else 0, None, out.data_ptr()], 6)
    return out


def release_stream(stream=None) -> None:
    L = _lib.load()
    s = stream if stream is not None else torch.cuda.current_stream()
    s.synchronize()
    L.tsdf_stream_release(s.cuda_stream)


def voxel_pixels(depth: torch.Tensor, offsets: torch.Tensor, headers: torch.Tensor, res: int = 32,
                 layout: str = "czyx", grid: Optional[torch.Tensor] = None, cam: Optional[_lib.TsdfCam] = None):
    L = _lib.load_debug()
    dev, n, R = _pack(L, depth, offsets, headers, res, layout)
    if grid is not None:
        _shaped("grid", grid, (n, 8), torch.float32, dev)
    tsdf = _out("tsdf", None, (n, 3, R, R, R), torch.float32, dev)
    pm = _out("pixmap", None, (n, R, R, R), torch.int32, dev)
    st = _out("status", None, (n,), torch.int32, dev)
    if n:
        _call(dev, L.tsdf_debug_pixmap_hip, _head(depth, offsets, headers, n, R, cam, layout) +
              [_ptr(grid), tsdf.data_ptr(), pm.data_ptr(), st.data_ptr()], 8)
    return tsdf, pm, st


class AabbBatch(NamedTuple):
    aabb: torch.Tensor
    grid: torch.Tensor
    ori: torch.Tensor
    status: torch.Tensor


def aabb(depth: torch.Tensor, offsets: torch.Tensor, headers: torch.Tensor, res: int = 32,
         cam: Optional[_lib.TsdfCam] = None) -> AabbBatch:
    L = _lib.load()
    dev, n, R = _pack(L, depth, offsets, headers, res)
    out = AabbBatch(_out("aabb", None, (n, 6), torch.float32, dev), _out("grid", None, (n, 8), torch.float32, dev),
                    _out("ori", None, (n, 3), torch.float32, dev), _out("status", None, (n,), torch.int32, dev))
    if n:
        _call(dev, L.tsdf_aabb_hip, [depth.data_ptr(), depth.numel(), offsets.data_ptr(), headers.data_ptr(), n, R, _cam(cam),
                                     None, out.aabb.data_ptr(), out.grid.data_ptr(), out.ori.data_ptr(),
                                     out.status.data_ptr()], 7)
    return out


def voxelize_grid(depth: torch.Tensor, offsets: torch.Tensor, headers: torch.Tensor, grid: torch.Tensor,
                  res: int = 32, layout: str = "czyx", cam: Optional[_lib.TsdfCam] = None):
    L = _lib.load()
    dev, n, R = _pack(L, depth, offsets, headers, res, layout)
    _shaped("grid", grid, (n, 8), torch.float32, dev)
    tsdf = _out("tsdf", None, (n, 3, R, R, R), torch.float32, dev)
    st = _out("status", None, (n,), torch.int32, dev)
    if n:
        _call(dev, L.tsdf_voxelize_grid_hip, _head(depth, offsets, headers, n, R, cam, layout) +
              [grid.data_ptr(), tsdf.data_ptr(), st.data_ptr()], 8)
    return tsdf, st


def voxelize_aug(depth: torch.Tensor, offsets: torch.Tensor, headers: torch.Tensor, xforms: torch.Tensor,
                 res: int = 64, layout: str = "czyx", cam: Optional[_lib.TsdfCam] = None,
                 out: Optional[TsdfBatch] = None, gt: Optional[torch.Tensor] = None, clamp: bool = True):
    L = _lib.load()
    dev, n, R = _pack(L, depth, offsets, headers, res, layout)
    _shaped("xforms", xforms, (n, 24), torch.float64, dev)
    out = _make_out(out, n, R, dev)
    lab = gt_nor = gt_aug = None
    if gt is not None:
        lab, gt_nor, gt_aug = _labels_struct(gt, n, n, dev, clamp, want_gt=True)
    if n:
        args = _head(depth, offsets, headers, n, R, cam, layout) + \
            [xforms.data_ptr(), out.tsdf.data_ptr(), out.max_l.data_ptr(), out.mid_p.data_ptr(), out.status.data_ptr()]
        if lab is None:
            _call(dev, L.tsdf_voxelize_aug_hip, args, 8)
        else:
            _call(dev, L.tsdf_voxelize_aug_labels_hip, args + [ctypes.byref(lab)], 8)
    return out if gt is None else (out, gt_nor, gt_aug)


_NO_STATE = object()


def _draw_args(centres, n, index, counters, out, params, state=_NO_STATE):
    _dev_check("centres", centres, torch.float32)
    dev = centres.device
    if centres.dim() != 2 or centres.shape[1] != 3:
        raise ValueError("centres must have shape [N, 3]")
    n_src = centres.shape[0]
    if state is not _NO_STATE:
        _dev_check("state", state, torch.int64, dev)
        if state.numel() != 2:
            raise ValueError("state must hold 2 elements: {key, counter0}")
    for name, t in (("index", index), ("counters", counters)):
        if t is None:
            continue
        _dev_check(name, t, torch.int64, dev, host_ok=True)
        if t.dim() != 1:
            raise ValueError(f"{name} must have shape [n]")
        if n is not None and int(n) != t.numel():
            raise ValueError(f"n must be the length of {name}" if t is index else "counters must have n entries")
        n = t.numel()
    n = n_src if n is None else int(n)
    if n < 0:
        raise ValueError("n must be >= 0")
    if n and n_src < 1:
        raise ValueError("centres holds no frame")
    xf = _out("out", out, (n, 24), torch.float64, dev)
    stretch = _out("stretch", None, (n,), torch.float64, dev) if params else None
    rot = _out("rot", None, (n, 2), torch.int32, dev) if params else None
    return dev, n_src, n, xf, stretch, rot


def aug_xforms(centres: torch.Tensor, n: Optional[int] = None, index: Optional[torch.Tensor] = None, key: int = 0,
               counter0: int = 0, out: Optional[torch.Tensor] = None, want_params: bool = False):
    A = _lib.load_augment()
    dev, n_src, n, xf, stretch, rot = _draw_args(centres, n, index, None, out, want_params)
    if n:
        m64 = (1 << 64) - 1
        _call(dev, A.tsdf_aug_draw_hip, [centres.data_ptr(), n_src, _ptr(index), n, int(key) & m64, int(counter0) & m64, None,
                                         xf.data_ptr(), _ptr(stretch), _ptr(rot)], 6)
    return (xf, stretch, rot) if want_params else xf


def _i64(v: int) -> int:
    v = int(v) & ((1 << 64) - 1)
    return v - (1 << 64) if v >> 63 else v


def aug_state(key: int, counter0: int = 0, device=None, out: Optional[torch.Tensor] = None) -> torch.Tensor:
    h = torch.tensor([_i64(key), _i64(counter0)], dtype=torch.int64)
    if out is None:
        return h.to(device)
    if out.dtype is not torch.int64 or out.numel() != 2:
        raise ValueError("state must be an int64 tensor of 2 elements")
    out.view(-1).copy_(h)
    return out


def aug_xforms_at(centres: torch.Tensor, state: torch.Tensor, n: Optional[int] = None,
                  index: Optional[torch.Tensor] = None, counters: Optional[torch.Tensor] = None,
                  out: Optional[torch.Tensor] = None, return_params: bool = False):
    A = _lib.load_augstep()
    dev, n_src, n, xf, stretch, rot = _draw_args(centres, n, index, counters, out, return_params, state)
    if n:
        _call(dev, A.tsdf_aug_draw_at_hip, [centres.data_ptr(), n_src, _ptr(index), n, state.data_ptr(), _ptr(counters), None,
                                            xf.data_ptr(), _ptr(stretch), _ptr(rot)], 6)
    return (xf, stretch, rot) if return_params else xf


class AugmentedStep:

    def __init__(self, depth: torch.Tensor, offsets: torch.Tensor, headers: torch.Tensor, n: int,
                 gt: Optional[torch.Tensor] = None, centres: Optional[torch.Tensor] = None, res: int = 32,
                 layout: str = "czyx", clamp: bool = True, cam: Optional[_lib.TsdfCam] = None, graph: bool = True,
                 dtype: Optional[torch.dtype] = None, base: Optional[torch.Tensor] = None, fused_head: bool = False):
        if graph not in (False, True):
            raise ValueError(f"graph must be False or True, got {graph!r}")
        if fused_head not in (False, True):
            raise ValueError(f"fused_head must be False or True, got {fused_head!r}")
        if dtype is not None:
            _lowp_dtype(dtype)
        self.dtype = dtype
        self.base = base
        self._head = bool(fused_head) or base is not None
        n = int(n)
        if n < 1:
            raise ValueError("n must be >= 1")
        dev, n_pack, R = _pack(_lib.load(), depth, offsets, headers, res, layout)
        self.n, self.res, self.layout, self.clamp, self.cam, self.device = n, R, layout, clamp, cam, dev
        self._pack_args = (depth, offsets, headers)
        self._gt = gt
        if base is not None:
            _shaped("base", base, (n_pack, 24), torch.float64, dev)
        if centres is not None:
            self.centres = centres
        elif base is not None:
            self.centres = map_grids(depth, offsets, headers, base, res=R, cam=cam).mid_p
        else:
            self.centres = aabb(depth, offsets, headers, res=R, cam=cam).grid[:, :3].contiguous()
        _shaped("centres", self.centres, (n_pack, 3), torch.float32, dev)
        self._in = torch.zeros(n + 2, dtype=torch.int64, device=dev)
        self.index, self.state = self._in[:n], self._in[n:]
        self._h = [torch.zeros(n + 2, dtype=torch.int64).pin_memory() for _ in range(2)]
        self._h_done = [None, None]
        self._turn = 0
        self.xforms = torch.empty((n, 24), dtype=torch.float64, device=dev)
        self.out = empty_batch(n, R, dev)
        if dtype is not None:
            self.out = self.out._replace(tsdf=torch.empty((n, 3, R, R, R), dtype=dtype, device=dev))
            self._grid = MapGridBatch(torch.empty((n, 8), dtype=torch.float32, device=dev), *self.out[1:])
        self.gt_nor = self.gt_aug = None
        if gt is not None:
            _dev_check("gt", gt, torch.float32, dev, host_ok=dtype is None)
            if dtype is not None and gt.shape[0] != n_pack:
                raise ValueError("gt must hold the labels of every frame of the pack: [N, 3*J] or [N, J, 3]")
            shape = (n,) + tuple(gt.shape[1:])
            self.gt_nor = torch.empty(shape, dtype=torch.float32, device=dev)
            self.gt_aug = torch.empty(shape, dtype=torch.float32, device=dev)
            if dtype is not None and not self._head:
                self._sel = (torch.empty(n, dtype=torch.int64, device=dev), torch.empty(shape, dtype=torch.float32, device=dev))
        if self._head:
            g = self._grid if dtype is not None else MapGridBatch(None, None, None, None)
            self._head_out = MapStepBatch(self.xforms, g.grid, g.max_l, g.mid_p, g.status, self.gt_aug, self.gt_nor)
        self.graph = None
        self._run()
        if graph:
            torch.cuda.synchronize(dev)
            side = torch.cuda.Stream(dev)
            g = torch.cuda.CUDAGraph()
            with torch.cuda.graph(g, stream=side):
                self._run()
            self.graph = g

    def _run(self):
        d, o, h = self._pack_args
        if self._head:
            lowp = self.dtype is not None
            map_step_head(d, o, h, self.centres, self.state, base=self.base, index=self.index,
                          gt=self._gt if lowp else None, res=self.res, cam=self.cam, clamp=self.clamp, place=lowp,
                          out=self._head_out)
            if lowp:
                _map_grid_lowp(d, o, h, self.xforms, self._grid.grid, self.res, self.layout, self.dtype, self.cam, self.index,
                               self.out.tsdf, False)
            else:
                voxelize_indexed(d, o, h, self.index, self._gt, res=self.res, layout=self.layout, cam=self.cam,
                                 clamp=self.clamp, out=self.out, xforms=self.xforms, out_gt_nor=self.gt_nor,
                                 out_gt=self.gt_aug)
            return
        aug_xforms_at(self.centres, self.state, index=self.index, out=self.xforms)
        if self.dtype is None:
            voxelize_indexed(d, o, h, self.index, self._gt, res=self.res, layout=self.layout, cam=self.cam, clamp=self.clamp,
                             out=self.out, xforms=self.xforms, out_gt_nor=self.gt_nor, out_gt=self.gt_aug)
            return
        map_grids(d, o, h, self.xforms, res=self.res, cam=self.cam, index=self.index, out=self._grid)
        _map_grid_lowp(d, o, h, self.xforms, self._grid.grid, self.res, self.layout, self.dtype, self.cam, self.index,
                       self.out.tsdf, False)
        if self._gt is not None:
            _batch_labels(self._gt, self.index, h.shape[0], self.xforms, self.out.max_l, self.out.mid_p, self.clamp,
                          sel=self._sel, out_aug=self.gt_aug, out_nor=self.gt_nor)

    def step(self, index, key: int, counter0: int = 0):
        n = self.n
        k = self._turn & 1
        self._turn += 1
        h = self._h[k]
        if self._h_done[k] is not None:
            self._h_done[k].synchronize()
        hn = h.numpy()
        hn[n] = _i64(key)
        hn[n + 1] = _i64(counter0)
        with _Current(self.device):
            if isinstance(index, torch.Tensor) and index.is_cuda:
                _shaped("index", index, (n,), torch.int64, self.device)
                self.index.copy_(index)
                self.state.copy_(h[n:], non_blocking=True)
            else:
                src = index.numpy() if isinstance(index, torch.Tensor) else index
                if len(src) != n:
                    raise ValueError(f"index must hold {n} frame numbers")
                hn[:n] = src
                self._in.copy_(h, non_blocking=True)
            if self._h_done[k] is None:
                self._h_done[k] = torch.cuda.Event()
            self._h_done[k].record(torch.cuda.current_stream(self.device))
            if self.graph is not None:
                self.graph.replay()
            else:
                self._run()
        return self.out if self._gt is None else (self.out, self.gt_nor, self.gt_aug)


class PointCloudBatch(NamedTuple):
    points: torch.Tensor
    count: torch.Tensor
    status: torch.Tensor


def point_clouds(depth: torch.Tensor, offsets: torch.Tensor, headers: torch.Tensor, points: int = 6000, seed: int = 0,
                 frame_base: int = 0, xforms: Optional[torch.Tensor] = None, cam: Optional[_lib.TsdfCam] = None,
                 out: Optional[PointCloudBatch] = None) -> PointCloudBatch:
    L = _lib.load()
    dev, n, _ = _pack(L, depth, offsets, headers)
    P = int(points)
    if not 1 <= P <= 0x7fffffff:
        raise ValueError("points must be in 1..2^31-1")
    seed, frame_base = int(seed), int(frame_base)
    if not 0 <= seed < 2 ** 64:
        raise ValueError("seed must be in [0, 2^64)")
    if not -2 ** 63 <= frame_base < 2 ** 63:
        raise ValueError("frame_base must fit int64")
    if xforms is not None:
        _shaped("xforms", xforms, (n, 24), torch.float64, dev)
    fields = (("points", (n, P, 3), torch.float64), ("count", (n,), torch.int32), ("status", (n,), torch.int32))
    if out is None:
        out = PointCloudBatch(*[_out(name, None, shape, dtype, dev) for name, shape, dtype in fields])
    else:
        for name, shape, dtype in fields:
            _shaped("out." + name, getattr(out, name), shape, dtype, dev)
    if n:
        _call(dev, L.tsdf_point_clouds_hip,
              [depth.data_ptr(), depth.numel(), offsets.data_ptr(), headers.data_ptr(), n, P, _cam(cam), seed, frame_base,
               _ptr(xforms), None, out.points.data_ptr(), out.count.data_ptr(), out.status.data_ptr()], 10)
    return out


class CloudGridBatch(NamedTuple):
    grid: torch.Tensor
    max_l: torch.Tensor
    mid_p: torch.Tensor
    aabb: torch.Tensor
    status: torch.Tensor


def cloud_grids(points: torch.Tensor, res: int = 32, cam: Optional[_lib.TsdfCam] = None) -> CloudGridBatch:
    L = _lib.load()
    _dev_check("points", points, torch.float64)
    dev = points.device
    if points.dim() != 3 or points.shape[2] != 3:
        raise ValueError("points must have shape [n, P, 3]")
    n, P = int(points.shape[0]), int(points.shape[1])
    if not 1 <= P <= 0x7fffffff:
        raise ValueError("points must hold 1..2^31-1 points per frame")
    if not L.tsdf_resolution_supported(int(res)):
        raise ValueError(f"unsupported grid resolution {res} (multiple of 4 in 4..128)")
    out = CloudGridBatch(_out("grid", None, (n, 8), torch.float32, dev), _out("max_l", None, (n,), torch.float32, dev),
                         _out("mid_p", None, (n, 3), torch.float32, dev), _out("aabb", None, (n, 6), torch.float32, dev),
                         _out("status", None, (n,), torch.int32, dev))
    if n:
        _call(dev, L.tsdf_cloud_grid_hip, [points.data_ptr(), n, P, int(res), _cam(cam), None, out.grid.data_ptr(),
                                           out.max_l.data_ptr(), out.mid_p.data_ptr(), out.aabb.data_ptr(),
                                           out.status.data_ptr()], 5)
    return out


class ProcessBatch(NamedTuple):
    points: torch.Tensor
    tsdf: torch.Tensor
    max_l: torch.Tensor
    mid_p: torch.Tensor
    status: torch.Tensor
    count: torch.Tensor


def process_batch(depth: torch.Tensor, offsets: torch.Tensor, headers: torch.Tensor, points: int = 6000, seed: int = 0,
                  frame_base: int = 0, res: int = 32, layout: str = "czyx",
                  cam: Optional[_lib.TsdfCam] = None, dtype: Optional[torch.dtype] = None) -> ProcessBatch:
    if dtype is not None:
        _lowp_dtype(dtype)
    pc = point_clouds(depth, offsets, headers, points=points, seed=seed, frame_base=frame_base, cam=cam)
    cg = cloud_grids(pc.points, res=res, cam=cam)
    if dtype is None:
        tsdf, st = voxelize_grid(depth, offsets, headers, cg.grid, res=res, layout=layout, cam=cam)
    else:
        tsdf, st = voxelize_grid_lowp(depth, offsets, headers, cg.grid, res=res, layout=layout, dtype=dtype, cam=cam)
    status = torch.where(pc.status != 0, pc.status, torch.where(cg.status != 0, cg.status, st))
    return ProcessBatch(pc.points, tsdf, cg.max_l, cg.mid_p, status, pc.count)


def voxelize_aug_grid(depth: torch.Tensor, offsets: torch.Tensor, headers: torch.Tensor, xforms: torch.Tensor,
                      grid: torch.Tensor, res: int = 32, layout: str = "czyx", cam: Optional[_lib.TsdfCam] = None):
    G = _lib.load_auggrid()
    dev, n, R = _pack(_lib.load(), depth, offsets, headers, res, layout)
    _shaped("xforms", xforms, (n, 24), torch.float64, dev)
    _shaped("grid", grid, (n, 8), torch.float32, dev)
    tsdf = _out("tsdf", None, (n, 3, R, R, R), torch.float32, dev)
    st = _out("status", None, (n,), torch.int32, dev)
    if n:
        _call(dev, G.tsdf_voxelize_aug_grid_hip, _head(depth, offsets, headers, n, R, cam, layout) +
              [xforms.data_ptr(), grid.data_ptr(), tsdf.data_ptr(), st.data_ptr()], 8)
    return tsdf, st


def transform_joints(gt: torch.Tensor, xforms: torch.Tensor, out: Optional[torch.Tensor] = None) -> torch.Tensor:
    G = _lib.load_auggrid()
    _dev_check("gt", gt, torch.float32)
    if gt.dim() < 2:
        raise ValueError("gt must have shape [n, 3*J] or [n, J, 3]")
    dev, n = gt.device, gt.shape[0]
    nc = _coords("gt", gt, n)
    _shaped("xforms", xforms, (n, 24), torch.float64, dev)
    out = _out("gt_aug", out, tuple(gt.shape), torch.float32, dev)
    if n:
        _call(dev, G.tsdf_transform_joints_hip, [gt.data_ptr(), xforms.data_ptr(), n, nc // 3, None, out.data_ptr()], 4)
    return out


class ProcessAugBatch(NamedTuple):
    points: torch.Tensor
    tsdf: torch.Tensor
    max_l: torch.Tensor
    mid_p: torch.Tensor
    points_aug: torch.Tensor
    tsdf_aug: torch.Tensor
    max_l_aug: torch.Tensor
    mid_p_aug: torch.Tensor
    gt_aug: Optional[torch.Tensor]
    status: torch.Tensor
    status_aug: torch.Tensor
    count: torch.Tensor
    xforms: torch.Tensor


def process_batch_aug(depth: torch.Tensor, offsets: torch.Tensor, headers: torch.Tensor,
                      xforms: Optional[torch.Tensor] = None, gt: Optional[torch.Tensor] = None, points: int = 6000,
                      seed: int = 0, aug_seed: int = 0, key: int = 0, frame_base: int = 0, res: int = 32,
                      layout: str = "czyx", cam: Optional[_lib.TsdfCam] = None,
                      dtype: Optional[torch.dtype] = None) -> ProcessAugBatch:
    if dtype is not None:
        _lowp_dtype(dtype)
    pb = process_batch(depth, offsets, headers, points=points, seed=seed, frame_base=frame_base, res=res, layout=layout,
                       cam=cam, dtype=dtype)
    if xforms is None:
        xforms = aug_xforms(pb.mid_p, key=key, counter0=frame_base)
    pa = point_clouds(depth, offsets, headers, points=points, seed=aug_seed, frame_base=frame_base, xforms=xforms, cam=cam)
    cg = cloud_grids(pa.points, res=res, cam=cam)
    if dtype is None:
        tsdf_aug, st = voxelize_aug_grid(depth, offsets, headers, xforms, cg.grid, res=res, layout=layout, cam=cam)
    else:
        tsdf_aug, st = voxelize_map_grid_lowp(depth, offsets, headers, xforms, cg.grid, res=res, layout=layout, dtype=dtype,
                                              cam=cam)
    status_aug = torch.where(pa.status != 0, pa.status, torch.where(cg.status != 0, cg.status, st))
    gt_aug = transform_joints(gt, xforms) if gt is not None else None
    return ProcessAugBatch(pb.points, pb.tsdf, pb.max_l, pb.mid_p, pa.points, tsdf_aug, cg.max_l, cg.mid_p, gt_aug,
                           pb.status, status_aug, pb.count, xforms)


def widen_depth16(src_u16: torch.Tensor, shift: int, out: Optional[torch.Tensor] = None) -> torch.Tensor:
    D = _lib.load_depth16()
    _dev_check("src_u16", src_u16, torch.uint16)
    if isinstance(shift, bool) or not isinstance(shift, int) or not 0 <= shift <= _lib.DEPTH16_MAX_SHIFT:
        raise ValueError(f"shift must be an integer in 0..{_lib.DEPTH16_MAX_SHIFT}, got {shift!r}")
    dev = src_u16.device
    out = _out("out", out, tuple(src_u16.shape), torch.float32, dev)
    if src_u16.numel():
        _call(dev, D.tsdf_depth16_widen_hip, [src_u16.data_ptr(), src_u16.numel(), shift, out.data_ptr(), None], 4)
    return out


class ObbBatch(NamedTuple):
    xforms: torch.Tensor
    status: torch.Tensor
    count: torch.Tensor
    mean: torch.Tensor
    cov: torch.Tensor
    eigenvalues: torch.Tensor


def obb_xforms(depth: torch.Tensor, offsets: torch.Tensor, headers: torch.Tensor, cam: Optional[_lib.TsdfCam] = None,
               out: Optional[torch.Tensor] = None) -> ObbBatch:
    O = _lib.load_obb()
    dev, n, _ = _pack(_lib.load(), depth, offsets, headers)
    xf = _out("out", out, (n, 24), torch.float64, dev)
    mo = _out("moments", None, (n, 16), torch.float64, dev)
    st = _out("status", None, (n,), torch.int32, dev)
    if n:
        _call(dev, O.tsdf_obb_xforms_hip, [depth.data_ptr(), depth.numel(), offsets.data_ptr(), headers.data_ptr(), n,
                                           _cam(cam), None, xf.data_ptr(), mo.data_ptr(), st.data_ptr()], 6)
    return ObbBatch(xf, st, mo[:, 0], mo[:, 1:4], mo[:, 4:10], mo[:, 10:13])


def voxelize_obb(depth: torch.Tensor, offsets: torch.Tensor, headers: torch.Tensor, res: int = 32, layout: str = "czyx",
                 cam: Optional[_lib.TsdfCam] = None, gt: Optional[torch.Tensor] = None, clamp: bool = True,
                 dtype: Optional[torch.dtype] = None):
    if dtype is not None:
        _lowp_dtype(dtype)
    xf = obb_xforms(depth, offsets, headers, cam=cam).xforms
    if dtype is None:
        r = voxelize_aug(depth, offsets, headers, xf, res=res, layout=layout, cam=cam, gt=gt, clamp=clamp)
    else:
        r = voxelize_aug_lowp(depth, offsets, headers, xf, res=res, layout=layout, dtype=dtype, cam=cam, gt=gt, clamp=clamp)
    return (r, xf) if gt is None else (r[0], r[1], r[2], xf)


def invert_xforms(xforms: torch.Tensor) -> torch.Tensor:
    if not isinstance(xforms, torch.Tensor):
        raise TypeError("xforms must be a torch.Tensor")
    if xforms.dim() != 2 or xforms.shape[1] != 24:
        raise ValueError("xforms must have shape [n, 24] (forward rows then inverse rows)")
    return torch.cat([xforms[:, 12:], xforms[:, :12]], dim=1)


_LOWP_DTYPES = {torch.float16: _lib.TSDF_LOWP_F16, torch.bfloat16: _lib.TSDF_LOWP_BF16}


def _lowp_dtype(dtype) -> int:
    code = _LOWP_DTYPES.get(dtype) if isinstance(dtype, torch.dtype) else None
    if code is None:
        raise ValueError(f"dtype must be torch.float16 or torch.bfloat16, got {dtype!r}")
    return code


def voxelize_grid_lowp(depth: torch.Tensor, offsets: torch.Tensor, headers: torch.Tensor, grid: torch.Tensor,
                       res: int = 32, layout: str = "czyx", dtype: torch.dtype = torch.bfloat16,
                       cam: Optional[_lib.TsdfCam] = None, index: Optional[torch.Tensor] = None,
                       out: Optional[torch.Tensor] = None):
    code = _lowp_dtype(dtype)
    P = _lib.load_lowp()
    dev, n_src, R = _pack(_lib.load(), depth, offsets, headers, res, layout)
    _shaped("grid", grid, (n_src, 8), torch.float32, dev)
    n = n_src
    if index is not None:
        _dev_check("index", index, torch.int64, dev)
        if index.dim() != 1:
            raise ValueError("index must have shape [n]")
        n = int(index.shape[0])
        if n and not n_src:
            raise ValueError("index needs at least one source frame")
    tsdf = _out("out", out, (n, 3, R, R, R), dtype, dev)
    st = _out("status", None, (n,), torch.int32, dev)
    if n:
        _call(dev, P.tsdf_voxelize_grid_lowp_hip,
              [depth.data_ptr(), depth.numel(), offsets.data_ptr(), headers.data_ptr(), n_src, _ptr(index), n, R, _cam(cam),
               _lib.LAYOUTS[layout], code, None, grid.data_ptr(), tsdf.data_ptr(), st.data_ptr()], 11)
    return tsdf, st


def voxelize_lowp(depth: torch.Tensor, offsets: torch.Tensor, headers: torch.Tensor, res: int = 32, layout: str = "czyx",
                  dtype: torch.dtype = torch.bfloat16, cam: Optional[_lib.TsdfCam] = None) -> TsdfBatch:
    _lowp_dtype(dtype)
    ab = aabb(depth, offsets, headers, res=res, cam=cam)
    rows = torch.cat([ab.ori, ab.grid[:, 4:6], torch.zeros_like(ab.ori)], dim=1)
    tsdf, _ = voxelize_grid_lowp(depth, offsets, headers, rows, res=res, layout=layout, dtype=dtype, cam=cam)
    return TsdfBatch(tsdf, ab.grid[:, 3].contiguous(), ab.grid[:, :3].contiguous(), ab.status)


def narrow_volumes(tsdf32: torch.Tensor, dtype: torch.dtype = torch.bfloat16,
                   out: Optional[torch.Tensor] = None) -> torch.Tensor:
    code = _lowp_dtype(dtype)
    P = _lib.load_lowp()
    _dev_check("tsdf32", tsdf32, torch.float32)
    dev = tsdf32.device
    out = _out("out", out, tuple(tsdf32.shape), dtype, dev)
    if tsdf32.numel():
        _call(dev, P.tsdf_lowp_narrow_hip, [tsdf32.data_ptr(), tsdf32.numel(), code, None, out.data_ptr()], 3)
    return out


class MapGridBatch(NamedTuple):
    grid: torch.Tensor
    max_l: torch.Tensor
    mid_p: torch.Tensor
    status: torch.Tensor


def _mapped(depth, offsets, headers, xforms, res, layout, index):
    dev, n_src, R = _pack(_lib.load(), depth, offsets, headers, res, layout)
    n = n_src
    if index is not None:
        _dev_check("index", index, torch.int64, dev)
        if index.dim() != 1:
            raise ValueError("index must have shape [n]")
        n = int(index.shape[0])
        if n and not n_src:
            raise ValueError("index needs at least one source frame")
    _shaped("xforms", xforms, (n, 24), torch.float64, dev)
    return dev, n_src, n, R


def map_grids(depth: torch.Tensor, offsets: torch.Tensor, headers: torch.Tensor, xforms: torch.Tensor, res: int = 32,
              cam: Optional[_lib.TsdfCam] = None, index: Optional[torch.Tensor] = None,
              out: Optional[MapGridBatch] = None) -> MapGridBatch:
    M = _lib.load_maplowp()
    dev, n_src, n, R = _mapped(depth, offsets, headers, xforms, res, "czyx", index)
    fields = (("grid", (n, 8), torch.float32), ("max_l", (n,), torch.float32), ("mid_p", (n, 3), torch.float32),
              ("status", (n,), torch.int32))
    if out is None:
        out = MapGridBatch(*[_out(name, None, shape, dtype, dev) for name, shape, dtype in fields])
    else:
        for name, shape, dtype in fields:
            _shaped("out." + name, getattr(out, name), shape, dtype, dev)
    if n:
        _call(dev, M.tsdf_map_place_hip,
              [depth.data_ptr(), depth.numel(), offsets.data_ptr(), headers.data_ptr(), n_src, _ptr(index), n, R, _cam(cam),
               None, xforms.data_ptr(), out.grid.data_ptr(), out.max_l.data_ptr(), out.mid_p.data_ptr(),
               out.status.data_ptr()], 9)
    return out


def _map_grid_lowp(depth, offsets, headers, xforms, grid, res, layout, dtype, cam, index, out, want_status):
    code = _lowp_dtype(dtype)
    M = _lib.load_maplowp()
    dev, n_src, n, R = _mapped(depth, offsets, headers, xforms, res, layout, index)
    _shaped("grid", grid, (n, 8), torch.float32, dev)
    tsdf = _out("out", out, (n, 3, R, R, R), dtype, dev)
    status = _out("status", None, (n,), torch.int32, dev) if want_status else None
    if n:
        _call(dev, M.tsdf_voxelize_map_grid_lowp_hip,
              [depth.data_ptr(), depth.numel(), offsets.data_ptr(), headers.data_ptr(), n_src, _ptr(index), n, R, _cam(cam),
               _lib.LAYOUTS[layout], code, None, xforms.data_ptr(), grid.data_ptr(), tsdf.data_ptr(), _ptr(status)], 11)
    return tsdf, status


def voxelize_map_grid_lowp(depth: torch.Tensor, offsets: torch.Tensor, headers: torch.Tensor, xforms: torch.Tensor,
                           grid: torch.Tensor, res: int = 32, layout: str = "czyx", dtype: torch.dtype = torch.bfloat16,
                           cam: Optional[_lib.TsdfCam] = None, index: Optional[torch.Tensor] = None,
                           out: Optional[torch.Tensor] = None):
    return _map_grid_lowp(depth, offsets, headers, xforms, grid, res, layout, dtype, cam, index, out, True)


def _batch_labels(gt, index, n_src, xforms, max_l, mid_p, clamp, sel=None, out_aug=None, out_nor=None):
    if index is not None:
        safe = index.clamp(0, n_src - 1) if sel is None else torch.clamp(index, 0, n_src - 1, out=sel[0])
        gt = gt.index_select(0, safe) if sel is None else torch.index_select(gt, 0, safe, out=sel[1])
    gt_aug = transform_joints(gt, xforms, out=out_aug)
    return normalize_joints(gt_aug, max_l, mid_p, clamp=clamp, out=out_nor), gt_aug


def voxelize_aug_lowp(depth: torch.Tensor, offsets: torch.Tensor, headers: torch.Tensor, xforms: torch.Tensor,
                      res: int = 32, layout: str = "czyx", dtype: torch.dtype = torch.bfloat16,
                      cam: Optional[_lib.TsdfCam] = None, gt: Optional[torch.Tensor] = None, clamp: bool = True,
                      index: Optional[torch.Tensor] = None):
    _lowp_dtype(dtype)
    mg = map_grids(depth, offsets, headers, xforms, res=res, cam=cam, index=index)
    tsdf, _ = _map_grid_lowp(depth, offsets, headers, xforms, mg.grid, res, layout, dtype, cam, index, None, False)
    batch = TsdfBatch(tsdf, mg.max_l, mg.mid_p, mg.status)
    if gt is None:
        return batch
    _dev_check("gt", gt, torch.float32, depth.device)
    gt_nor, gt_aug = _batch_labels(gt, index, headers.shape[0], xforms, mg.max_l, mg.mid_p, clamp)
    return batch, gt_nor, gt_aug


def compose_xforms(outer: torch.Tensor, inner: torch.Tensor, index: Optional[torch.Tensor] = None,
                   out: Optional[torch.Tensor] = None) -> torch.Tensor:
    S = _lib.load_mapstep()
    _dev_check("outer", outer, torch.float64)
    dev = outer.device
    if outer.dim() != 2 or outer.shape[1] != 24:
        raise ValueError("outer must have shape [n, 24] (forward rows then inverse rows)")
    n = outer.shape[0]
    _dev_check("inner", inner, torch.float64, dev)
    if inner.dim() != 2 or inner.shape[1] != 24:
        raise ValueError("inner must have shape [N, 24] (forward rows then inverse rows)")
    n_inner = inner.shape[0]
    if index is not None:
        _shaped("index", index, (n,), torch.int64, dev)
        if n and not n_inner:
            raise ValueError("index needs at least one inner map")
    elif n_inner != n:
        raise ValueError("without index, inner must hold one map per map of outer")
    out = _out("out", out, (n, 24), torch.float64, dev)
    if n:
        _call(dev, S.tsdf_compose_xforms_hip, [outer.data_ptr(), inner.data_ptr(), n_inner, _ptr(index), n, None,
                                               out.data_ptr()], 5)
    return out


class MapStepBatch(NamedTuple):
    xforms: torch.Tensor
    grid: Optional[torch.Tensor]
    max_l: Optional[torch.Tensor]
    mid_p: Optional[torch.Tensor]
    status: Optional[torch.Tensor]
    gt_aug: Optional[torch.Tensor]
    gt_nor: Optional[torch.Tensor]


def map_step_head(depth: torch.Tensor, offsets: torch.Tensor, headers: torch.Tensor, centres: torch.Tensor,
                  state: torch.Tensor, *, base: Optional[torch.Tensor] = None, index: Optional[torch.Tensor] = None,
                  counters: Optional[torch.Tensor] = None, gt: Optional[torch.Tensor] = None, res: int = 32,
                  cam: Optional[_lib.TsdfCam] = None, clamp: bool = True, place: bool = True,
                  out: Optional[MapStepBatch] = None, return_params: bool = False):
    S = _lib.load_mapstep()
    dev, n_src, R = _pack(_lib.load(), depth, offsets, headers, res)
    _, n_c, n, xf, stretch, rot = _draw_args(centres, None, index, counters, out.xforms if out is not None else None,
                                             return_params, state)
    if centres.device != dev:
        raise ValueError(f"centres is on {centres.device}, expected {dev}")
    if n_c != n_src:
        raise ValueError("centres must hold one centre per source frame: [N, 3]")
    if base is not None:
        _shaped("base", base, (n_src, 24), torch.float64, dev)
    grid = max_l = mid_p = status = gt_aug = gt_nor = None
    nj = 0
    if place:
        fields = (("grid", (n, 8), torch.float32), ("max_l", (n,), torch.float32), ("mid_p", (n, 3), torch.float32),
                  ("status", (n,), torch.int32))
        grid, max_l, mid_p, status = (_out("out." + name, getattr(out, name) if out is not None else None, shape, dtype, dev)
                                      for name, shape, dtype in fields)
    if gt is not None:
        if not place:
            raise ValueError("gt needs place=True (the labels are normalised in the placed grid)")
        _dev_check("gt", gt, torch.float32, dev)
        if gt.dim() < 2:
            raise ValueError("gt must hold the labels of every source frame: [N, 3*J] or [N, J, 3]")
        nj = (_coords("gt", gt, n_src) or 63) // 3
        shape = (n,) + tuple(gt.shape[1:])
        gt_aug = _out("out.gt_aug", out.gt_aug if out is not None else None, shape, torch.float32, dev)
        gt_nor = _out("out.gt_nor", out.gt_nor if out is not None else None, shape, torch.float32, dev)
    if n:
        c = cam if cam is not None else _lib.default_cam()
        _call(dev, S.tsdf_map_step_head_hip,
              [depth.data_ptr(), depth.numel(), offsets.data_ptr(), headers.data_ptr(), n_src, _ptr(index), n, R, c.focal, c.cx,
               c.cy, c.invalid_eps, c.trunc_voxels, centres.data_ptr(), _ptr(base), state.data_ptr(), _ptr(counters), _ptr(gt), nj,
               1 if clamp else 0, None,
               xf.data_ptr(), _ptr(grid), _ptr(max_l), _ptr(mid_p), _ptr(status), _ptr(gt_aug), _ptr(gt_nor), _ptr(stretch),
               _ptr(rot)], 20)
    batch = MapStepBatch(xf, grid, max_l, mid_p, status, gt_aug, gt_nor)
    return (batch, stretch, rot) if return_params else batch


class HandCrops(NamedTuple):
    depth: torch.Tensor
    offsets: torch.Tensor
    headers: torch.Tensor
    com: torch.Tensor
    count: torch.Tensor
    status: torch.Tensor
    grid: Optional[torch.Tensor]
    max_l: Optional[torch.Tensor]
    mid_p: Optional[torch.Tensor]


_LOCATE_TYPES = {torch.float32: _lib.TSDF_LOCATE_F32, torch.uint16: _lib.TSDF_LOCATE_U16}


def locate_hands(frames: torch.Tensor, *, cube: float = 250.0, near: float = 100.0, far: float = 1500.0,
                 seed_band: float = 150.0, refine: int = 2, res: int = 32, cam: Optional[_lib.TsdfCam] = None,
                 shift: Optional[int] = None, index: Optional[torch.Tensor] = None, grid: bool = True,
                 out: Optional[HandCrops] = None) -> HandCrops:
    K = _lib.load_locate()
    if not isinstance(frames, torch.Tensor):
        raise TypeError("frames must be a torch.Tensor")
    if frames.dtype not in _LOCATE_TYPES:
        raise TypeError(f"frames must be torch.float32 or torch.uint16, got {frames.dtype}")
    if frames.dim() != 3 or frames.shape[1] < 1 or frames.shape[2] < 1:
        raise ValueError("frames must have shape [N, H, W]")
    u16 = frames.dtype is torch.uint16
    if u16:
        if isinstance(shift, bool) or not isinstance(shift, int) or not 0 <= shift <= _lib.DEPTH16_MAX_SHIFT:
            raise ValueError(f"uint16 frames need shift, an integer in 0..{_lib.DEPTH16_MAX_SHIFT}; got {shift!r}")
    elif shift is not None:
        raise ValueError("shift belongs to uint16 frames")
    if not _lib.load().tsdf_resolution_supported(int(res)):
        raise ValueError(f"unsupported grid resolution {res} (multiple of 4 in 4..128)")
    if isinstance(refine, bool) or not isinstance(refine, int):
        raise TypeError("refine must be an integer")
    if not frames.is_contiguous():
        raise ValueError("frames must be contiguous")
    _dev_check("frames", frames, frames.dtype)
    dev = frames.device
    n_src, H, W = (int(v) for v in frames.shape)
    n = n_src
    if index is not None:
        _dev_check("index", index, torch.int64, dev)
        if index.dim() != 1:
            raise ValueError("index must have shape [n]")
        n = int(index.shape[0])
        if n and not n_src:
            raise ValueError("index needs at least one frame")
    c = cam if cam is not None else _lib.default_cam()
    per = ctypes.c_int64(0)
    _lib.check(K.tsdf_locate_capacity(H, W, cube, near, c.focal, ctypes.byref(per)), "tsdf_locate_capacity")
    need = n * per.value
    get = (lambda name: getattr(out, name)) if out is not None else (lambda name: None)
    if out is not None:
        _dev_check("out.depth", out.depth, torch.float32, dev)
        if out.depth.dim() != 1 or out.depth.numel() < need:
            raise ValueError(f"out.depth must be a vector of at least {need} elements ({n} frames of {per.value})")
        depth = out.depth
    else:
        depth = torch.empty((need,), dtype=torch.float32, device=dev)
    if n == 0:
        offsets = torch.zeros((1,), dtype=torch.int64, device=dev) if out is None else \
            _shaped("out.offsets", out.offsets, (1,), torch.int64, dev).zero_()
    else:
        offsets = _out("out.offsets", get("offsets"), (n + 1,), torch.int64, dev)
    headers = _out("out.headers", get("headers"), (n, 6), torch.int32, dev)
    com = _out("out.com", get("com"), (n, 3), torch.float64, dev)
    count = _out("out.count", get("count"), (n,), torch.int32, dev)
    status = _out("out.status", get("status"), (n,), torch.int32, dev)
    g = max_l = mid_p = None
    if grid:
        g = _out("out.grid", get("grid"), (n, 8), torch.float32, dev)
        max_l = _out("out.max_l", get("max_l"), (n,), torch.float32, dev)
        mid_p = _out("out.mid_p", get("mid_p"), (n, 3), torch.float32, dev)
    if n:
        _call(dev, K.tsdf_locate_hip,
              [frames.data_ptr(), _LOCATE_TYPES[frames.dtype], shift if u16 else 0, n_src, H, W, _ptr(index), n, near, far, cube,
               seed_band, refine, int(res), c.focal, c.cx, c.cy, c.invalid_eps, c.trunc_voxels, depth.numel(), None,
               depth.data_ptr(), offsets.data_ptr(), headers.data_ptr(), com.data_ptr(), count.data_ptr(), status.data_ptr(),
               _ptr(g), _ptr(max_l), _ptr(mid_p)], 20)
    return HandCrops(depth, offsets, headers, com, count, status, g, max_l, mid_p)


def voxelize_frames(frames: torch.Tensor, res: int = 32, *, placement: str = "aabb", dtype: Optional[torch.dtype] = None,
                    gt: Optional[torch.Tensor] = None, layout: str = "czyx", **locate):
    if placement not in ("aabb", "cube"):
        raise ValueError("placement must be 'aabb' or 'cube'")
    if layout not in _lib.LAYOUTS:
        raise ValueError("layout must be 'czyx' or 'cxyz'")
    if dtype is not None:
        _lowp_dtype(dtype)
    if "grid" in locate or "res" in locate:
        raise TypeError("voxelize_frames sets locate_hands' grid and res itself")
    cam = locate.get("cam")
    crops = locate_hands(frames, res=res, grid=placement == "cube", **locate)
    d, o, h = crops.depth, crops.offsets, crops.headers
    gt_nor = None
    if placement == "aabb":
        if dtype is not None:
            batch = voxelize_lowp(d, o, h, res=res, layout=layout, dtype=dtype, cam=cam)
        elif gt is not None:
            batch, gt_nor = voxelize_labels(d, o, h, gt, res=res, layout=layout, cam=cam)
        else:
            batch = voxelize(d, o, h, res=res, layout=layout, cam=cam)
    else:
        if dtype is not None:
            tsdf, st = voxelize_grid_lowp(d, o, h, crops.grid, res=res, layout=layout, dtype=dtype, cam=cam)
        else:
            tsdf, st = voxelize_grid(d, o, h, crops.grid, res=res, layout=layout, cam=cam)
        batch = TsdfBatch(tsdf, crops.max_l, crops.mid_p, st)
    if gt is None:
        return batch, crops
    if gt_nor is None:
        gt_nor = normalize_joints(gt, batch.max_l, batch.mid_p)
    return batch, crops, gt_nor
```

Baseline: 7.260 million.

## Precompute per-frame grid tables once and voxelize resident packs with new f32 kernel

```diff
diff --git a/handposeestimation-with-3d-cnns_amd/__init__.py b/handposeestimation-with-3d-cnns_amd/__init__.py
--- a/handposeestimation-with-3d-cnns_amd/__init__.py
+++ b/handposeestimation-with-3d-cnns_amd/__init__.py
@@ -8,7 +8,7 @@
                        voxelize, voxelize_aug, voxelize_grid, voxelize_indexed, voxelize_labels, widen_depth16,
                        invert_xforms, obb_xforms, voxelize_obb, narrow_volumes, voxelize_grid_lowp, voxelize_lowp,
                        map_grids, voxelize_aug_lowp, voxelize_map_grid_lowp, MapStepBatch, compose_xforms, map_step_head,
-                       HandCrops, locate_hands, voxelize_frames)
+                       HandCrops, locate_hands, voxelize_frames, ResidentGrid, resident_grid, voxelize_resident)
 from .pca import JointPCA, fit_joint_pca
 from . import augment, dataset, export, packing, pca, shard, synth
 from .dataset import MSRA_Dataset, MSRADepthDataset, ResidentLoader, VoxelBatch, VoxelLoader
@@ -25,4 +25,4 @@
            "ProcessAugBatch", "widen_depth16", "obb_xforms", "voxelize_obb", "invert_xforms", "ObbBatch",
            "voxelize_grid_lowp", "voxelize_lowp", "narrow_volumes", "map_grids", "MapGridBatch", "voxelize_map_grid_lowp",
            "voxelize_aug_lowp", "compose_xforms", "map_step_head", "MapStepBatch", "locate_hands", "voxelize_frames",
-           "HandCrops"]
+           "HandCrops", "ResidentGrid", "resident_grid", "voxelize_resident"]
diff --git a/handposeestimation-with-3d-cnns_amd/_lib.py b/handposeestimation-with-3d-cnns_amd/_lib.py
--- a/handposeestimation-with-3d-cnns_amd/_lib.py
+++ b/handposeestimation-with-3d-cnns_amd/_lib.py
@@ -104,6 +104,9 @@
 TSDF_LOCATE_F32 = 0
 TSDF_LOCATE_U16 = 1
 
+GRIDF32_LIB_PATH = os.path.join(_HERE, "libtsdf_gridf32.so")
+GRIDF32_VERSION = 1
+
 
 class _Ext(NamedTuple):
     path: str
@@ -155,6 +158,12 @@
                             ctypes.c_float, _i64, _vp, _vp, _vp, _vp, _vp, _vp, _vp, _vp, _vp, _vp],
     }),
 }
+
+_GRIDF32 = _Ext(GRIDF32_LIB_PATH, "tsdf_gridf32_version", GRIDF32_VERSION, {
+    "tsdf_voxelize_grid_f32_hip": [_vp, _i64, _vp, _vp, _i64, _vp, _i, _i, ctypes.c_double, ctypes.c_double, ctypes.c_double,
+                                   ctypes.c_float, ctypes.c_float, _i, _vp, _vp, _vp, _vp, _vp, _vp, _vp, _vp,
+                                   ctypes.POINTER(TsdfLabels)],
+})
 
 _lib = None
 _debug_lib = None
@@ -245,7 +254,7 @@
     L = _ext_libs.get(name)
     if L is not None:
         return L
-    ext = _EXTS[name]
+    ext = _GRIDF32 if name == "gridf32" else _EXTS[name]
     if not os.path.exists(ext.path):
         raise ImportError(f"{ext.path} not found: build it with `make -C handposeestimation-with-3d-cnns_amd/csrc "
                           f"{name}` (__graft_entry__.build() does). There is no CPU fallback.")
@@ -294,6 +303,10 @@
     return _load_ext("locate")
 
 
+def load_gridf32():
+    return _load_ext("gridf32")
+
+
 @contextlib.contextmanager
 def using_debug_library():
     global _lib
diff --git a/handposeestimation-with-3d-cnns_amd/csrc/gridf32_host.inc b/handposeestimation-with-3d-cnns_amd/csrc/gridf32_host.inc
--- /dev/null
+++ b/handposeestimation-with-3d-cnns_amd/csrc/gridf32_host.inc
@@ -0,0 +1,58 @@
+
+constexpr int kGridF32WG = 256;
+constexpr int kGridF32Items = 1024;
+constexpr int kGridF32Tab = 256;
+#ifndef TSDF_GRIDF32_WG_PER_CU
+#define TSDF_GRIDF32_WG_PER_CU 4
+#endif
+
+struct GridF32Plan {
+  int chunk;
+  int slab;
+  int nslab;
+  int64_t blocks;
+};
+
+inline bool gridf32_plan(int n, int R, int cus, GridF32Plan &p) {
+  const int per = R * (R / 4);
+  p.chunk = (kGridF32Items + per - 1) / per;
+  if (p.chunk > R) p.chunk = R;
+  const int finest = (R + p.chunk - 1) / p.chunk;
+  int64_t want = finest;
+  if (cus > 0 && n > 0) {
+    want = ((int64_t)cus * TSDF_GRIDF32_WG_PER_CU + n - 1) / n;
+    if (want > finest) want = finest;
+  }
+  const int chunks = (int)((finest + want - 1) / want);
+  p.slab = chunks * p.chunk;
+  if (p.slab > R) p.slab = R;
+  p.nslab = (R + p.slab - 1) / p.slab;
+  p.blocks = (int64_t)n * p.nslab;
+  return p.blocks * kGridF32WG <= 0xffffffffll;
+}
+
+struct GridF32Call {
+  const void *depth, *offsets, *headers, *index, *grid, *ori, *src_status, *out_tsdf;
+  int64_t depth_len, n_src;
+  int n, R, layout;
+  const tsdf_cam *cam;
+  const tsdf_labels *labels;
+};
+
+inline int gridf32_check(const GridF32Call &c, GridF32Plan &plan, bool *run) {
+  *run = false;
+  if (c.n < 0) return TSDF_ERR_INVALID_ARG;
+  if (c.R < 4 || c.R > 128 || c.R % 4 != 0) return TSDF_ERR_INVALID_ARG;
+  if (c.layout != TSDF_LAYOUT_CZYX && c.layout != TSDF_LAYOUT_CXYZ) return TSDF_ERR_INVALID_ARG;
+  if (c.labels && (c.labels->n_joints < 1 || c.labels->n_joints > 170)) return TSDF_ERR_INVALID_ARG;
+  if (c.n == 0) return TSDF_OK;
+  if (!c.depth || !c.offsets || !c.headers || !c.grid || !c.ori || !c.src_status || !c.out_tsdf || c.depth_len < 0)
+    return TSDF_ERR_INVALID_ARG;
+  if (c.n_src < 1 || (!c.index && c.n_src != c.n)) return TSDF_ERR_INVALID_ARG;
+  if (reinterpret_cast<uintptr_t>(c.out_tsdf) & 15) return TSDF_ERR_INVALID_ARG;
+  if (c.labels && (!c.labels->d_gt || !c.labels->d_out_gt_nor)) return TSDF_ERR_INVALID_ARG;
+  if (!cam_ok(c.cam)) return TSDF_ERR_INVALID_ARG;
+  if (!gridf32_plan(c.n, c.R, 0, plan)) return TSDF_ERR_INVALID_ARG;
+  *run = true;
+  return TSDF_OK;
+}
diff --git a/handposeestimation-with-3d-cnns_amd/csrc/gridf32_host_main.cc b/handposeestimation-with-3d-cnns_amd/csrc/gridf32_host_main.cc
--- /dev/null
+++ b/handposeestimation-with-3d-cnns_amd/csrc/gridf32_host_main.cc
@@ -0,0 +1,148 @@
+#include <stdint.h>
+#include <stdio.h>
+
+#include <initializer_list>
+
+#include "../../include/tsdf_gridf32.h"
+
+namespace {
+#define TSDF_PRIM_HOST_ONLY
+#include "prim.inc"
+#include "gridf32_host.inc"
+
+int failures = 0;
+void expect(bool ok, const char *what, int line) {
+  if (!ok) {
+    fprintf(stderr, "gridf32_host_main.cc:%d: %s\n", line, what);
+    ++failures;
+  }
+}
+#define EXPECT(c) expect((c), #c, __LINE__)
+
+GridF32Call good(char *mem) {
+  GridF32Call c;
+  c.depth = c.offsets = c.headers = c.grid = c.ori = c.src_status = mem;
+  c.index = nullptr;
+  c.out_tsdf = mem;
+  c.depth_len = 100, c.n_src = 1;
+  c.n = 1, c.R = 32, c.layout = TSDF_LAYOUT_CZYX;
+  c.cam = nullptr, c.labels = nullptr;
+  return c;
+}
+
+int check(const GridF32Call &c, bool *run = nullptr, GridF32Plan *plan = nullptr) {
+  GridF32Plan p = {-1, -1, -1, -1};
+  bool r = true;
+  const int rc = gridf32_check(c, p, &r);
+  if (run) *run = r;
+  if (plan) *plan = p;
+  if (rc != TSDF_OK) EXPECT(!r);
+  return rc;
+}
+}
+
+int main() {
+  alignas(16) static char mem[64];
+  for (int R = 4; R <= 128; R += 4) {
+    GridF32Plan fine;
+    EXPECT(gridf32_plan(3, R, 0, fine));
+    for (int cus : {0, 1, 8, 256, 304}) {
+      for (int n : {1, 3, 16, 300, 1024, 100000}) {
+        GridF32Plan p;
+        EXPECT(gridf32_plan(n, R, cus, p));
+        EXPECT(p.chunk == fine.chunk && p.chunk >= 1 && p.chunk * R <= kGridF32Tab);
+        EXPECT(p.slab >= p.chunk && p.slab <= R && (p.slab % p.chunk == 0 || p.slab == R));
+        EXPECT(p.nslab == (R + p.slab - 1) / p.slab && p.blocks == (int64_t)n * p.nslab);
+        EXPECT((int64_t)(p.nslab - 1) * p.slab < R && (int64_t)p.nslab * p.slab >= R);
+        EXPECT(p.nslab >= 1 && p.nslab <= fine.nslab);
+        if (cus == 0) EXPECT(p.nslab == fine.nslab);
+      }
+    }
+    const int per = R * (R / 4);
+    EXPECT(fine.chunk == 1 || (fine.chunk - 1) * per < kGridF32Items);
+  }
+  {
+    GridF32Plan p;
+    EXPECT(gridf32_plan(1024, 32, 0, p) && p.chunk == 4 && p.slab == 4 && p.nslab == 8 && p.blocks == 8192);
+    EXPECT(gridf32_plan(1024, 32, 256, p) && p.chunk == 4 && p.slab == 32 && p.nslab == 1 && p.blocks == 1024);
+    EXPECT(gridf32_plan(512, 32, 256, p) && p.slab == 16 && p.nslab == 2 && p.blocks == 1024);
+    EXPECT(gridf32_plan(16, 32, 256, p) && p.slab == 4 && p.nslab == 8);
+    EXPECT(gridf32_plan(100000, 32, 256, p) && p.slab == 32 && p.nslab == 1);
+    EXPECT(gridf32_plan(1, 12, 256, p) && p.slab == 12 && p.nslab == 1);
+    EXPECT(gridf32_plan(1, 64, 0, p) && p.slab == 1 && p.nslab == 64);
+    EXPECT(gridf32_plan((1 << 17) - 1, 128, 0, p));
+    EXPECT(!gridf32_plan(1 << 17, 128, 0, p));
+    EXPECT(!gridf32_plan(0x7fffffff, 128, 0, p));
+    EXPECT(gridf32_plan(0x7fffffff / 512, 8, 0, p));
+  }
+  bool run = false;
+  GridF32Plan plan;
+  GridF32Call c = good(mem);
+  EXPECT(check(c, &run, &plan) == TSDF_OK && run && plan.blocks == 8);
+  c.n = -1;
+  EXPECT(check(c) == TSDF_ERR_INVALID_ARG);
+  c = good(mem), c.n = 0, c.n_src = 0;
+  c.depth = c.offsets = c.headers = c.grid = c.ori = c.src_status = c.out_tsdf = nullptr;
+  EXPECT(check(c, &run) == TSDF_OK && !run);
+  c.R = 30;
+  EXPECT(check(c) == TSDF_ERR_INVALID_ARG);
+  for (int R : {0, 2, 3, 6, 30, 132, 256, -4}) {
+    c = good(mem), c.R = R;
+    EXPECT(check(c) == TSDF_ERR_INVALID_ARG);
+  }
+  for (int layout : {-1, 2}) {
+    c = good(mem), c.layout = layout;
+    EXPECT(check(c) == TSDF_ERR_INVALID_ARG);
+  }
+  const void *GridF32Call::*ptrs[] = {&GridF32Call::depth, &GridF32Call::offsets, &GridF32Call::headers, &GridF32Call::grid,
+                                      &GridF32Call::ori, &GridF32Call::src_status, &GridF32Call::out_tsdf};
+  for (auto m : ptrs) {
+    c = good(mem), c.*m = nullptr;
+    EXPECT(check(c) == TSDF_ERR_INVALID_ARG);
+  }
+  c = good(mem), c.depth_len = -1;
+  EXPECT(check(c) == TSDF_ERR_INVALID_ARG);
+  c = good(mem), c.n_src = 0, c.index = mem;
+  EXPECT(check(c) == TSDF_ERR_INVALID_ARG);
+  c = good(mem), c.n_src = 2;
+  EXPECT(check(c) == TSDF_ERR_INVALID_ARG);
+  c.index = mem;
+  EXPECT(check(c, &run) == TSDF_OK && run);
+  c = good(mem), c.out_tsdf = mem + 8;
+  EXPECT(check(c) == TSDF_ERR_INVALID_ARG);
+  tsdf_labels lab = {reinterpret_cast<const float *>(mem), 21, 1, reinterpret_cast<float *>(mem), nullptr};
+  c = good(mem), c.labels = &lab;
+  EXPECT(check(c, &run) == TSDF_OK && run);
+  for (int j : {0, -1, 171}) {
+    lab.n_joints = j;
+    EXPECT(check(c) == TSDF_ERR_INVALID_ARG);
+    c.n = 0;
+    EXPECT(check(c) == TSDF_ERR_INVALID_ARG);
+    c.n = 1;
+  }
+  lab.n_joints = 170, lab.d_gt = nullptr;
+  EXPECT(check(c) == TSDF_ERR_INVALID_ARG);
+  lab.d_gt = reinterpret_cast<const float *>(mem), lab.d_out_gt_nor = nullptr;
+  EXPECT(check(c) == TSDF_ERR_INVALID_ARG);
+  c.n = 0;
+  EXPECT(check(c, &run) == TSDF_OK && !run);
+  tsdf_cam cam = {241.42, 160.0, 120.0, 1.0f, 3.0f};
+  c = good(mem), c.cam = &cam;
+  EXPECT(check(c, &run) == TSDF_OK && run);
+  cam.focal = 0.0;
+  EXPECT(check(c) == TSDF_ERR_INVALID_ARG);
+  cam.focal = 241.42, cam.invalid_eps = -1.0f;
+  EXPECT(check(c) == TSDF_ERR_INVALID_ARG);
+  cam.invalid_eps = 1.0f, cam.trunc_voxels = 0.0f / 1.0f * 0.0f;
+  EXPECT(check(c) == TSDF_ERR_INVALID_ARG);
+  c = good(mem), c.n = c.n_src = 1 << 17, c.R = 128;
+  EXPECT(check(c) == TSDF_ERR_INVALID_ARG);
+  c.n = c.n_src = (1 << 17) - 1;
+  EXPECT(check(c, &run, &plan) == TSDF_OK && run && plan.blocks == ((1ll << 17) - 1) * 128);
+  if (failures) {
+    fprintf(stderr, "%d check(s) failed\n", failures);
+    return 1;
+  }
+  printf("gridf32 host checks passed\n");
+  return 0;
+}
diff --git a/handposeestimation-with-3d-cnns_amd/csrc/tsdf_gridf32.hip b/handposeestimation-with-3d-cnns_amd/csrc/tsdf_gridf32.hip
--- /dev/null
+++ b/handposeestimation-with-3d-cnns_amd/csrc/tsdf_gridf32.hip
@@ -0,0 +1,325 @@
+
+#include <hip/hip_runtime.h>
+#include <stdint.h>
+#include <string.h>
+
+#include <atomic>
+
+#include "../../include/tsdf_gridf32.h"
+
+namespace {
+
+#pragma clang diagnostic push
+#pragma clang diagnostic ignored "-Wunused-function"
+#include "device.inc"
+#include "prim.inc"
+#include "slab.inc"
+#pragma clang diagnostic pop
+#include "gridf32_host.inc"
+
+static_assert(kGridF32WG == kSlabWG, "the plan and the scaffold agree on the workgroup");
+
+typedef float gf_f4 __attribute__((ext_vector_type(4)));
+typedef __attribute__((address_space(1))) float *GlobalOutF;
+
+#ifndef TSDF_GRIDF32_STORE_ASM
+#define TSDF_GRIDF32_STORE_ASM "sc1 nt"
+#endif
+__device__ __forceinline__ void store_vol4(GlobalOutF p, gf_f4 v) {
+  asm volatile("global_store_dwordx4 %0, %1, off " TSDF_GRIDF32_STORE_ASM "\n\ts_nop 1" ::"v"(p), "v"(v) : "memory");
+}
+
+struct GridF32Args {
+  const float *depth;
+  int64_t depth_len;
+  const int64_t *offsets;
+  const int32_t *headers;
+  int64_t n_src;
+  const int64_t *index;
+  int n, R;
+  int slab;
+  int nslab;
+  int chunk;
+  double focal, cx, cy, inv_focal;
+  float eps;
+  const float *grid;
+  const float *ori;
+  const int32_t *src_status;
+  float *out;
+  float *max_l;
+  float *mid_p;
+  int32_t *status;
+  const float *gt;
+  float *gt_nor, *gt_aug;
+  int n_joints, clamp;
+};
+
+typedef int gf_i4 __attribute__((ext_vector_type(4)));
+
+template <int LAYOUT, bool POW2>
+__global__ __launch_bounds__(kSlabWG) void tsdf_grid_f32_kernel(GridF32Args a) {
+#pragma clang fp contract(off)
+  constexpr int V = 4;
+  __shared__ double s_vx[kSlabMaxR], s_vxs[kSlabMaxR];
+  __shared__ double s_nvy[kSlabMaxR], s_vys[kSlabMaxR];
+  __shared__ double s_q[kSlabMaxR], s_vzs[kSlabMaxR];
+  __shared__ float s_neg[kSlabMaxR];
+  __shared__ alignas(16) int t_px[kGridF32Tab];
+  __shared__ alignas(16) int t_py[kGridF32Tab];
+
+  const int tid = threadIdx.x;
+  const int R = a.R, RV = R / V;
+  const Slab blk = slab_of_block(a.nslab, a.slab, R);
+  const int64_t i = blk.i;
+  const int sb = blk.sb, se = blk.se;
+  const int64_t R3 = (int64_t)R * R * R;
+  float *__restrict__ out = a.out + i * 3 * R3;
+
+  const int64_t g = a.index ? a.index[i] : i;
+  const bool src_ok = g >= 0 && g < a.n_src;
+  const int64_t gs = src_ok ? g : 0, depth_len = a.depth_len;
+  const int32_t *hd = a.headers + 6 * gs;
+  const int left = hd[2], top = hd[3], right = hd[4], bottom = hd[5];
+  const int64_t off0 = a.offsets[gs], off1 = a.offsets[gs + 1];
+  const int64_t bw = (int64_t)right - left;
+  const bool hdr_ok = src_ok && header_ok(left, top, right, bottom, off0, off1, depth_len);
+  const float *gr = a.grid + 8 * gs, *go = a.ori + 3 * gs;
+  const float ox = go[0], oy = go[1], oz = go[2], vl = gr[4], td = gr[5];
+  const int tab_status = a.src_status[gs];
+  const bool grid_ok = td > 0.0f && finite32(td) && finite32(vl) && finite32(ox) && finite32(oy) && finite32(oz);
+  const int status = !hdr_ok ? TSDF_FRAME_BAD_HEADER
+                             : tab_status != TSDF_FRAME_OK ? tab_status : !grid_ok ? TSDF_FRAME_DEGENERATE : TSDF_FRAME_OK;
+  const float max_l = hdr_ok ? gr[3] : 0.0f;
+  const float mid0 = hdr_ok ? gr[0] : 0.0f, mid1 = hdr_ok ? gr[1] : 0.0f, mid2 = hdr_ok ? gr[2] : 0.0f;
+
+  if (blk.first()) {
+    if (tid == 0) {
+      if (a.status) a.status[i] = status;
+      if (a.max_l) a.max_l[i] = max_l;
+      if (a.mid_p) {
+        a.mid_p[3 * i + 0] = mid0;
+        a.mid_p[3 * i + 1] = mid1;
+        a.mid_p[3 * i + 2] = mid2;
+      }
+    }
+    if (a.gt) {
+      const int nc = 3 * a.n_joints;
+      for (int e = tid; e < nc; e += kSlabWG) {
+        const int c = e % 3;
+        const float v = a.gt[gs * nc + e];
+        if (a.gt_aug) a.gt_aug[i * nc + e] = v;
+        float o = 0.5f;
+        if (status == TSDF_FRAME_OK) {
+          const float m = c == 0 ? mid0 : (c == 1 ? mid1 : mid2);
+          o = __fadd_rn(__fdiv_rn(__fsub_rn(v, m), max_l), 0.5f);
+          if (a.clamp) {
+            o = o < 0.f ? 0.f : o;
+            o = o > 1.f ? 1.f : o;
+          }
+        }
+        a.gt_nor[i * nc + e] = o;
+      }
+    }
+  }
+
+  if (status != TSDF_FRAME_OK) {
+    slab_zero_fill<gf_f4>(out, R, sb, (int64_t)(se - sb) * R * R / 4, tid);
+    return;
+  }
+
+  const double F = a.focal, cx = a.cx, cy = a.cy;
+  const double it = 1.0 / (double)td;
+  const double kq = a.inv_focal * it;
+  for (int e = tid; e < 3 * R; e += kSlabWG) {
+    const int ax = e / R, idx = e - ax * R;
+    const float o = ax == 0 ? ox : ax == 1 ? oy : oz;
+    const double prod = (double)idx * (double)vl;
+    const double v = (double)o + prod;
+    const double vs = v * it;
+    if (ax == 0) {
+      s_vx[idx] = v;
+      s_vxs[idx] = vs;
+    } else if (ax == 1) {
+      s_nvy[idx] = -v;
+      s_vys[idx] = vs;
+    } else {
+      s_q[idx] = -F / v;
+      s_vzs[idx] = vs;
+      s_neg[idx] = f32_round_up(-v);
+    }
+  }
+  const float eps = a.eps;
+  const float *__restrict__ d = a.depth + off0;
+  const int lgR = POW2 ? __builtin_ctz((unsigned)R) : 0, lgRV = POW2 ? lgR - 2 : 0;
+  for (int cb = sb; cb < se; cb += a.chunk) {
+  const int ce = cb + a.chunk < se ? cb + a.chunk : se;
+  __syncthreads();
+  const int ns = ce - cb;
+  for (int e = tid; e < ns * R; e += kSlabWG) {
+    const int s = e / R, k = e - s * R;
+    if constexpr (LAYOUT == 0) {
+      const double q = s_q[cb + s];
+      const double mx = s_vx[k] * q, my = s_nvy[k] * q;
+      const int px = trunc_i32(mx + cx), py = trunc_i32(my + cy);
+      t_px[e] = px >= left && px < right ? px - left : -1;
+      t_py[e] = py >= top && py < bottom ? py - top : -1;
+    } else {
+      const double mx = s_vx[cb + s] * s_q[k];
+      const int px = trunc_i32(mx + cx);
+      t_px[e] = px >= left && px < right ? px - left : -1;
+    }
+  }
+  __syncthreads();
+
+  const int nit = ns * R * RV;
+  for (int item = tid; item < nit; item += kSlabWG) {
+    int fq, y, s;
+    if constexpr (POW2) {
+      fq = item & (RV - 1);
+      const int t1 = item >> lgRV;
+      y = t1 & (R - 1);
+      s = t1 >> lgR;
+    } else {
+      fq = item % RV;
+      const int t1 = item / RV;
+      y = t1 % R;
+      s = t1 / R;
+    }
+    const int fv = fq * V, sl = cb + s;
+    const double vys = s_vys[y];
+    const gf_i4 rx4 = *reinterpret_cast<const gf_i4 *>(&t_px[s * R + fv]);
+    const int rx[V] = {rx4.x, rx4.y, rx4.z, rx4.w};
+    int ry[V];
+    if constexpr (LAYOUT == 0) {
+      ry[0] = ry[1] = ry[2] = ry[3] = t_py[s * R + y];
+    } else {
+      const double nvy = s_nvy[y];
+#pragma unroll
+      for (int j = 0; j < V; ++j) {
+        const double my = nvy * s_q[fv + j];
+        const int py = trunc_i32(my + cy);
+        ry[j] = py >= top && py < bottom ? py - top : -1;
+      }
+    }
+    float pd[V];
+    bool inb[V];
+#pragma unroll
+    for (int j = 0; j < V; ++j) {
+      inb[j] = (rx[j] | ry[j]) >= 0;
+      const int64_t at = inb[j] ? (int64_t)ry[j] * bw + rx[j] : 0;
+      pd[j] = d[at];
+    }
+    double pd64[V], tz[V];
+    float sv[V];
+    bool any_near = false;
+#pragma unroll
+    for (int j = 0; j < V; ++j) {
+      const int zi = LAYOUT == 0 ? sl : fv + j;
+      const bool ok = inb[j] & (__builtin_fabsf(pd[j]) >= eps);
+      pd64[j] = (double)pd[j];
+      tz[j] = __builtin_fma(pd64[j], it, s_vzs[zi]);
+      const bool neg = pd[j] < s_neg[zi];
+      any_near |= ok & (__builtin_fabs(tz[j]) <= 1.0);
+      sv[j] = ok ? (neg ? -1.0f : 1.0f) : 0.0f;
+    }
+    gf_f4 o0 = {sv[0], sv[1], sv[2], sv[3]}, o1 = o0, o2 = o0;
+    if (__any(any_near)) {
+#pragma unroll
+      for (int j = 0; j < V; ++j) {
+        const int xi = LAYOUT == 0 ? fv + j : sl;
+        const double aq = pd64[j] * kq;
+        const double dxi = (double)(rx[j] + left) - cx, dyi = (double)(ry[j] + top) - cy;
+        const double tx = __builtin_fma(-dxi, aq, s_vxs[xi]);
+        const double ty = __builtin_fma(dyi, aq, vys);
+        const double xx = tx * tx;
+        const double sq = __builtin_fma(tz[j], tz[j], __builtin_fma(ty, ty, xx));
+        const bool nearv = sq <= 1.0;
+        const float m0 = __builtin_fminf(__builtin_fabsf((float)tx), 1.0f);
+        const float m1 = __builtin_fminf(__builtin_fabsf((float)ty), 1.0f);
+        const float m2 = __builtin_fminf(__builtin_fabsf((float)tz[j]), 1.0f);
+        o0[j] = nearv ? m0 * sv[j] : sv[j];
+        o1[j] = nearv ? m1 * sv[j] : sv[j];
+        o2[j] = nearv ? m2 * sv[j] : sv[j];
+      }
+    }
+    const int64_t e = ((int64_t)sl * R + y) * R + fv;
+    store_vol4((GlobalOutF)(out + e), o0);
+    store_vol4((GlobalOutF)(out + R3 + e), o1);
+    store_vol4((GlobalOutF)(out + 2 * R3 + e), o2);
+  }
+  }
+}
+
+template <int LAYOUT>
+void launch_grid(const GridF32Args &a, int64_t blocks, hipStream_t s) {
+  if ((a.R & (a.R - 1)) == 0)
+    hipLaunchKernelGGL((tsdf_grid_f32_kernel<LAYOUT, true>), dim3((unsigned)blocks), dim3(kSlabWG), 0, s, a);
+  else
+    hipLaunchKernelGGL((tsdf_grid_f32_kernel<LAYOUT, false>), dim3((unsigned)blocks), dim3(kSlabWG), 0, s, a);
+}
+
+}
+
+extern "C" {
+
+int tsdf_gridf32_version(void) { return TSDF_GRIDF32_VERSION; }
+
+int tsdf_voxelize_grid_f32_hip(const float *d_depth, int64_t depth_len, const int64_t *d_offsets,
+                               const int32_t *d_headers, int64_t n_src, const int64_t *d_index, int n, int R,
+                               double focal, double cx, double cy, float invalid_eps, float trunc_voxels, int layout,
+                               void *hip_stream, const float *d_grid,
+                               const float *d_ori, const int32_t *d_src_status, float *d_out_tsdf, float *d_out_max_l,
+                               float *d_out_mid_p, int32_t *d_out_status, const tsdf_labels *labels) {
+  const tsdf_cam cam_v = {focal, cx, cy, invalid_eps, trunc_voxels};
+  const tsdf_cam *cam = &cam_v;
+  GridF32Call c;
+  c.depth = d_depth, c.offsets = d_offsets, c.headers = d_headers, c.index = d_index;
+  c.grid = d_grid, c.ori = d_ori, c.src_status = d_src_status, c.out_tsdf = d_out_tsdf;
+  c.depth_len = depth_len, c.n_src = n_src;
+  c.n = n, c.R = R, c.layout = layout;
+  c.cam = cam, c.labels = labels;
+  GridF32Plan plan;
+  bool run;
+  const int bad = gridf32_check(c, plan, &run);
+  if (bad != TSDF_OK || !run) return bad;
+  const int cus = device_cus();
+  if (cus < 0) return cus;
+  gridf32_plan(n, R, cus, plan);
+  GridF32Args a;
+  a.depth = d_depth;
+  a.depth_len = depth_len;
+  a.offsets = d_offsets;
+  a.headers = d_headers;
+  a.n_src = n_src;
+  a.index = d_index;
+  a.n = n;
+  a.R = R;
+  a.slab = plan.slab;
+  a.nslab = plan.nslab;
+  a.chunk = plan.chunk;
+  a.focal = cam->focal;
+  a.cx = cam->cx;
+  a.cy = cam->cy;
+  a.inv_focal = 1.0 / cam->focal;
+  a.eps = cam->invalid_eps;
+  a.grid = d_grid;
+  a.ori = d_ori;
+  a.src_status = d_src_status;
+  a.out = d_out_tsdf;
+  a.max_l = d_out_max_l;
+  a.mid_p = d_out_mid_p;
+  a.status = d_out_status;
+  a.gt = labels ? labels->d_gt : nullptr;
+  a.gt_nor = labels ? labels->d_out_gt_nor : nullptr;
+  a.gt_aug = labels ? labels->d_out_gt_aug : nullptr;
+  a.n_joints = labels ? labels->n_joints : 0;
+  a.clamp = labels ? labels->clamp : 0;
+  hipStream_t s = static_cast<hipStream_t>(hip_stream);
+  if (layout == TSDF_LAYOUT_CZYX)
+    launch_grid<0>(a, plan.blocks, s);
+  else
+    launch_grid<1>(a, plan.blocks, s);
+  return launched();
+}
+
+}
diff --git a/handposeestimation-with-3d-cnns_amd/dataset.py b/handposeestimation-with-3d-cnns_amd/dataset.py
--- a/handposeestimation-with-3d-cnns_amd/dataset.py
+++ b/handposeestimation-with-3d-cnns_amd/dataset.py
@@ -16,7 +16,8 @@
 from .pca import JointPCA, fit_joint_pca
 from .voxelize import (AugmentedStep, TsdfBatch, _get_raw_stream, aabb, aug_state, aug_xforms, aug_xforms_at,
                        denormalize_joints, empty_batch, normalize_joints, obb_xforms, project_joints, voxelize,
-                       voxelize_aug, voxelize_grid_lowp, voxelize_indexed, voxelize_labels, widen_depth16, _lowp_dtype)
+                       voxelize_aug, voxelize_grid_lowp, voxelize_indexed, voxelize_labels, widen_depth16, _lowp_dtype,
+                       resident_grid, voxelize_resident)
 
 
 def _common_depth_shift(packs: Sequence[packing.PackedFrames]) -> Optional[int]:
@@ -417,7 +418,7 @@
                  seed: int = 0, drop_last: bool = False, rank: int = 0, world: int = 1, labels: bool = True,
                  clamp: bool = True, layout: str = "czyx", augment: Union[bool, str] = False, balance: str = "frames",
                  prefetch: int = 1, ring: int = 2, graph: bool = False, frame: str = "camera",
-                 volume_dtype: Optional[torch.dtype] = None):
+                 volume_dtype: Optional[torch.dtype] = None, plan: bool = False):
         if frame not in ("camera", "obb"):
             raise ValueError(f"frame must be 'camera' or 'obb', got {frame!r}")
         if frame == "obb" and (augment or graph):
@@ -445,6 +446,8 @@
         self.obb_status = None
         self._step = None
         self.volume_dtype = volume_dtype
+        self.planned = bool(plan) and volume_dtype is None and not augment and frame == "camera" and not graph
+        self._grid = None
         self._lowp = None
         self._lowp_ring = None
         self._mapped = self.augment or frame == "obb"
@@ -464,6 +467,7 @@
         self._dev = (rp.depth, rp.offsets, rp.headers, rp.gt)
         self._g = rp.frame
         pin = self.bs > _lib.INLINE_INDEX_MAX or self._mapped
+        self._pin = pin
         self._idx = [(torch.empty(self.bs, dtype=torch.int64).pin_memory() if pin else torch.empty(self.bs, dtype=torch.int64),
                       torch.cuda.Event()) for _ in range(2)]
         self._used = [False, False]
@@ -471,8 +475,9 @@
         if self.frame == "obb":
             ob = obb_xforms(rp.depth, rp.offsets, rp.headers)
             self.obb, self.obb_status = ob.xforms, ob.status
+        if self.planned or self.volume_dtype is not None:
+            ab = self._grid = resident_grid(rp.depth, rp.offsets, rp.headers, res=self.res)
         if self.volume_dtype is not None:
-            ab = aabb(rp.depth, rp.offsets, rp.headers, res=self.res)
             rows = torch.cat([ab.ori, ab.grid[:, 4:6], torch.zeros_like(ab.ori)], dim=1)
             self._lowp = (rows, ab.grid[:, 3].contiguous(), ab.grid[:, :3].contiguous(), ab.status)
         if self.augment:
@@ -574,8 +579,12 @@
                         h_xf.numpy()[:n] = self._host_draw(gidx, (b,), epoch, k)
                         drawn = h_xf[:n].to(self.device, non_blocking=True)
                     xf = self._maps(idx, k & 1, key, pos, drawn)
-                out, gt_nor, g = voxelize_indexed(depth, off, hdr, idx, gt, res=self.res, layout=self.layout,
-                                                  clamp=self.clamp, gt_copy=True, xforms=xf)
+                if self.planned and self._pin:
+                    out, gt_nor, g = voxelize_resident(depth, off, hdr, self._grid, idx, gt, layout=self.layout,
+                                                       clamp=self.clamp, gt_copy=True)
+                else:
+                    out, gt_nor, g = voxelize_indexed(depth, off, hdr, idx, gt, res=self.res, layout=self.layout,
+                                                      clamp=self.clamp, gt_copy=True, xforms=xf)
                 done.record(cur)
                 self._used[k & 1] = True
             pos += n
@@ -626,8 +635,12 @@
             idx, xf = d_idx[pos:pos + nfr], None
             if self._mapped:
                 xf = self._maps(idx, blk % self.ring, key, pos, None if d_xf is None else d_xf[pos:pos + nfr])
-            voxelize_indexed(depth, off, hdr, idx, gt, res=self.res, layout=self.layout, clamp=self.clamp,
-                             out=o, out_gt_nor=gn, out_gt=gg, xforms=xf)
+            if self.planned:
+                voxelize_resident(depth, off, hdr, self._grid, idx, gt, layout=self.layout, clamp=self.clamp,
+                                  out=o, out_gt_nor=gn, out_gt=gg)
+            else:
+                voxelize_indexed(depth, off, hdr, idx, gt, res=self.res, layout=self.layout, clamp=self.clamp,
+                                 out=o, out_gt_nor=gn, out_gt=gg, xforms=xf)
             pos += nfr
             if full:
                 yield from views
@@ -711,7 +724,8 @@
 
     def __init__(self, root_path, opt=None, train=True, aug=False, device="cuda", block: int = 1024,
                  packed_dir: Optional[str] = None, resident: Optional[bool] = None, prebatched: Optional[bool] = None,
-                 ring: Optional[int] = None, aug_seed: int = 0, _raw: Optional[MSRADepthDataset] = None, pca=None):
+                 ring: Optional[int] = None, aug_seed: int = 0, _raw: Optional[MSRADepthDataset] = None, pca=None,
+                 plan: bool = False):
         if isinstance(aug, str) and aug != "device":
             raise ValueError(f"aug must be False, True or 'device', got {aug!r}")
         self.AUG = bool(aug)
@@ -735,6 +749,8 @@
             raise ValueError("prebatched=True needs a resident (pack-backed) dataset")
         self._ring_req = ring
         self._rp: Optional[ResidentPacks] = None
+        self._plan = bool(plan)
+        self._grid = None
         self._fast = None
         self._n = len(self.raw)
         self._aug_params = None
@@ -772,6 +788,8 @@
     def _resident_packs(self) -> "ResidentPacks":
         if self._rp is None:
             self._rp = ResidentPacks(self.raw, self.device)
+            if self._plan and not self.AUG and self.pca is None:
+                self._grid = resident_grid(self._rp.depth, self._rp.offsets, self._rp.headers)
             if self.AUG:
                 rp = self._rp
                 mid = aabb(rp.depth, rp.offsets, rp.headers).grid[:, :3]
@@ -807,6 +825,10 @@
             elif self.AUG:
                 xf = torch.from_numpy(self._xf_table[idx]).to(dev)
             frame = self._frame2 if self.AUG else rp.frame
+            if self._grid is not None:
+                r = voxelize_resident(rp.depth, rp.offsets, rp.headers, self._grid, torch.from_numpy(frame[idx]).to(dev),
+                                      rp.gt, clamp=clamp, gt_copy=True)
+                return r[0], r[2], r[1], None
             r = voxelize_indexed(rp.depth, rp.offsets, rp.headers, torch.from_numpy(frame[idx]).to(dev), rp.gt,
                                  clamp=clamp, gt_copy=True, xforms=xf, **kw)
             return r[0], r[2], r[1], (r[3] if kw else None)
@@ -871,7 +893,7 @@
         pca, k = None, 0
 
         def __init__(self, rp: "ResidentPacks", bs: int, ring: int, device, frame=None, xf_table=None, pca=None, k=0,
-                     draw=None):
+                     draw=None, grid=None):
             self._ctypes, self._lib = ctypes, _lib
             self.always_fresh = not _slot_guard_works()
             ring = max(2, int(ring))
@@ -905,8 +927,15 @@
             self.cur_dev = getattr(torch._C, "_cuda_getDevice", torch.cuda.current_device)
             self.fn = self.L.tsdf_voxelize_indexed_hip
             self.plain_xf = ()
+            self.cam_args = (None,)
             if pca is not None:
                 self.fn, self.plain_xf = self.L.tsdf_voxelize_indexed_pca_hip, (None,)
+            elif grid is not None:
+                self.grid = grid
+                self.fn = _lib.load_gridf32().tsdf_voxelize_grid_f32_hip
+                c = _lib.default_cam()
+                self.cam_args = (c.focal, c.cx, c.cy, c.invalid_eps, c.trunc_voxels)
+                self.plain_xf = (grid.grid.data_ptr(), grid.ori.data_ptr(), grid.status.data_ptr())
             self.take = (rp.frame if frame is None else frame).take
             self.by_value = xf_table is None and draw is None and bs <= _lib.INLINE_INDEX_MAX
             self.fn_host = self.L.tsdf_voxelize_indexed_host_hip if pca is None else \
@@ -990,7 +1019,7 @@
                 f.sync()
             f = self._fast = MSRA_Dataset._Fast(self._rp, n, self._ring_size(n), self.device,
                                                 frame=self._frame2 if self.AUG else None, xf_table=self._xf_table,
-                                                pca=self.pca, k=self.PCA_SZ,
+                                                pca=self.pca, k=self.PCA_SZ, grid=self._grid,
                                                 draw=(self._aug_mid, self._device_state(), self._draw_frame,
                                                       self._draw_counter) if self.aug_device else None)
         k = f.next_slot()
@@ -1036,10 +1065,10 @@
             else:
                 fn = f.fn
                 if f.cur_dev() == f.dev_index:
-                    rc = fn(*f.head, f.idx_ptrs[ki], n, 32, None, 0, f.raw_stream(f.dev_index), *f.plain_xf, *a)
+                    rc = fn(*f.head, f.idx_ptrs[ki], n, 32, *f.cam_args, 0, f.raw_stream(f.dev_index), *f.plain_xf, *a)
                 else:
                     with torch.cuda.device(f.device):
-                        rc = fn(*f.head, f.idx_ptrs[ki], n, 32, None, 0, f.raw_stream(f.dev_index), *f.plain_xf, *a)
+                        rc = fn(*f.head, f.idx_ptrs[ki], n, 32, *f.cam_args, 0, f.raw_stream(f.dev_index), *f.plain_xf, *a)
             if within == f.kGroup - 1:
                 f.read[ki >> 4].record(torch.cuda.current_stream(f.device))
                 f.read_used[ki >> 4] = True
diff --git a/handposeestimation-with-3d-cnns_amd/voxelize.py b/handposeestimation-with-3d-cnns_amd/voxelize.py
--- a/handposeestimation-with-3d-cnns_amd/voxelize.py
+++ b/handposeestimation-with-3d-cnns_amd/voxelize.py
@@ -378,6 +378,68 @@
                                      None, out.aabb.data_ptr(), out.grid.data_ptr(), out.ori.data_ptr(),
                                      out.status.data_ptr()], 7)
     return out
+
+
+_default_cam_values = None
+
+
+def _cam_values(cam) -> tuple:
+    global _default_cam_values
+    if cam is None:
+        if _default_cam_values is None:
+            c = _lib.default_cam()
+            _default_cam_values = (c.focal, c.cx, c.cy, c.invalid_eps, c.trunc_voxels)
+        return _default_cam_values
+    return (cam.focal, cam.cx, cam.cy, cam.invalid_eps, cam.trunc_voxels)
+
+
+class ResidentGrid(NamedTuple):
+    grid: torch.Tensor
+    ori: torch.Tensor
+    status: torch.Tensor
+    res: int
+
+
+def resident_grid(depth: torch.Tensor, offsets: torch.Tensor, headers: torch.Tensor, res: int = 32,
+                  cam: Optional[_lib.TsdfCam] = None) -> ResidentGrid:
+    ab = aabb(depth, offsets, headers, res=res, cam=cam)
+    return ResidentGrid(ab.grid, ab.ori, ab.status, int(res))
+
+
+def voxelize_resident(depth: torch.Tensor, offsets: torch.Tensor, headers: torch.Tensor, tables: ResidentGrid,
+                      index: Optional[torch.Tensor] = None, gt: Optional[torch.Tensor] = None, layout: str = "czyx",
+                      cam: Optional[_lib.TsdfCam] = None, clamp: bool = True, out: Optional[TsdfBatch] = None,
+                      gt_copy: bool = False, out_gt_nor: Optional[torch.Tensor] = None,
+                      out_gt: Optional[torch.Tensor] = None):
+    P = _lib.load_gridf32()
+    dev, n_pack, R = _pack(_lib.load(), depth, offsets, headers, tables.res, layout)
+    _shaped("tables.grid", tables.grid, (n_pack, 8), torch.float32, dev)
+    _shaped("tables.ori", tables.ori, (n_pack, 3), torch.float32, dev)
+    _shaped("tables.status", tables.status, (n_pack,), torch.int32, dev)
+    n = n_pack
+    if index is not None:
+        _dev_check("index", index, torch.int64, dev, host_ok=True)
+        if index.dim() != 1:
+            raise ValueError("index must have shape [n]")
+        n = int(index.shape[0])
+        if n and not n_pack:
+            raise ValueError("index needs at least one source frame")
+    out = _make_out(out, n, R, dev)
+    lab = gt_nor = gt_dev = None
+    if gt is not None:
+        if gt.dim() < 2:
+            raise ValueError("gt must hold the labels of every frame of the pack: [N, 3*J] or [N, J, 3]")
+        lab, gt_nor, gt_dev = _labels_struct(gt, n_pack, n, dev, clamp, out_gt_nor, out_gt, want_gt=gt_copy)
+        gt_copy = gt_dev is not None
+    if n:
+        _call(dev, P.tsdf_voxelize_grid_f32_hip,
+              [depth.data_ptr(), depth.numel(), offsets.data_ptr(), headers.data_ptr(), n_pack, _ptr(index), n, R,
+               *_cam_values(cam), _lib.LAYOUTS[layout], None, tables.grid.data_ptr(), tables.ori.data_ptr(), tables.status.data_ptr(),
+               out.tsdf.data_ptr(), out.max_l.data_ptr(), out.mid_p.data_ptr(), out.status.data_ptr(),
+               ctypes.byref(lab) if lab is not None else None], 14)
+    if gt is None:
+        return out
+    return (out, gt_nor, gt_dev) if gt_copy else (out, gt_nor)
 
 
 def voxelize_grid(depth: torch.Tensor, offsets: torch.Tensor, headers: torch.Tensor, grid: torch.Tensor,
diff --git a/include/tsdf_gridf32.h b/include/tsdf_gridf32.h
--- /dev/null
+++ b/include/tsdf_gridf32.h
@@ -0,0 +1,27 @@
+#ifndef TSDF_GRIDF32_H_
+#define TSDF_GRIDF32_H_
+
+#include <stdint.h>
+
+#include "tsdf.h"
+
+#ifdef __cplusplus
+extern "C" {
+#endif
+
+#define TSDF_GRIDF32_VERSION 1
+
+int tsdf_gridf32_version(void);
+
+int tsdf_voxelize_grid_f32_hip(const float *d_depth, int64_t depth_len, const int64_t *d_offsets,
+                               const int32_t *d_headers, int64_t n_src, const int64_t *d_index, int n, int R,
+                               double focal, double cx, double cy, float invalid_eps, float trunc_voxels, int layout,
+                               void *hip_stream, const float *d_grid,
+                               const float *d_ori, const int32_t *d_src_status, float *d_out_tsdf, float *d_out_max_l,
+                               float *d_out_mid_p, int32_t *d_out_status, const tsdf_labels *labels);
+
+#ifdef __cplusplus
+}
+#endif
+
+#endif
```

Measured after the change: 7.258 million. Within noise of the previous version (-0.0%).
